# RainbowZL0/swin-unet-image-fusion

Hardware: AMD Instinct MI355X
Metric: fused image-pairs/sec at 256x256, win=8 (higher is better)
Workload: dtype bf16; 1 GPU; B=16/GPU 256x256 IR/visible pairs, win=8, 5-level Swin-UNet fusion forward (BASELINE configs[1]); global_batch=16, precision_mode=fast, residual_stream=fp32, hip_graph=True, steps_in_flight=3, kernel_schedule=throughput, collective=none, weights=random-init (numpy PCG64 recipe, seed 0)

## Files before the change

### swin_unet_image_fusion_amd/csrc/kernels_mlp.h

```cpp
#pragma once
#include "kernels_deep.h"

namespace swf {

struct MlpFusedDesc {
    const float* x[2];
    float* out[2];
    const float* gamma[2]; const float* beta[2];
    const bf16_raw* w1_hi[2]; const bf16_raw* w1_lo[2];
    const bf16_raw* w2_hi[2]; const bf16_raw* w2_lo[2];
    const float* b1[2]; const float* b2[2];
    float* scratch; int64_t scratch_floats;
    int M, C, HID;
    int schedule;
    const float* ln_gamma[2]; const float* ln_beta[2]; bf16_raw* ln_hi[2]; bf16_raw* ln_lo[2];
    const float* part0[2]; const float* part1[2]; const float* pbias[2]; float* x1[2];
};

bool mlp_fused_supported(int C, int HID);
int mlp_fused_splits(int C, int HID);
inline bool mlp_fused_writes_ln(int, int) { return true; }
int launch_mlp_fused(const MlpFusedDesc& d, int nstream, hipStream_t stream, int* route = nullptr);

}
```

### swin_unet_image_fusion_amd/csrc/kernels_mlp.hip

```cpp
#include "kernels_mlp.h"

#include <algorithm>
#include <cstdlib>

#include "win_frag.h"

#ifdef SWF_MLP_PROBE
__device__ unsigned long long swf_mlp_probe[64];
__device__ unsigned long long swf_mlp_wg[2 * 4096];
#define SWF_PROBE(i) do { if (threadIdx.x == 0) { const unsigned long long t_ = wall_clock64(); \
        if (blockIdx.x == SWF_MLP_PROBE && blockIdx.y == 0 && blockIdx.z == 0) swf_mlp_probe[i] = t_; \
        if ((i) == 0 || (i) == 41) swf_mlp_wg[2 * (((blockIdx.z * gridDim.y + blockIdx.y) * gridDim.x + blockIdx.x) & 4095) + ((i) == 41)] = t_; } } while (0)
#else
#define SWF_PROBE(i) do { } while (0)
#endif

namespace swf {

namespace {

using namespace wf;

struct MlpArgs {
    const float* x[2]; float* out[2];
    const float* gamma[2]; const float* beta[2];
    const bf16* w1_hi[2]; const bf16* w1_lo[2]; const bf16* w2_hi[2]; const bf16* w2_lo[2];
    const float* b1[2]; const float* b2[2];
    float* scratch;
    int M, HID, splits, nchunks;
    const float* ln_gamma[2]; const float* ln_beta[2]; bf16* ln_hi[2]; bf16* ln_lo[2];
    const float* part0[2]; const float* part1[2]; const float* pbias[2]; float* x1[2];
};

__device__ __forceinline__ void mma3(f32x16& acc, const bf16x8 wh, const bf16x8 wl, const bf16x8 bh, const bf16x8 bl) {
    acc = __builtin_amdgcn_mfma_f32_32x32x16_bf16(wl, bh, acc, 0, 0, 0);
    acc = __builtin_amdgcn_mfma_f32_32x32x16_bf16(wh, bl, acc, 0, 0, 0);
    acc = __builtin_amdgcn_mfma_f32_32x32x16_bf16(wh, bh, acc, 0, 0, 0);
}

template <int C, int NW, int TOK = 64>
__global__ __launch_bounds__(64 * NW) void mlp_fused_kernel(MlpArgs a) {
    constexpr int NT = 64 * NW, CW = 32 * NW;
    constexpr int NTT = TOK / 32;
    static_assert(TOK == 32 || TOK == 64, "token tile");
    constexpr int TPR = (NT / TOK == 4 || NT / TOK == 8) ? NT / TOK : 8;
    constexpr int LNT = TOK * TPR;
    static_assert(LNT <= NT, "row threads");
    constexpr int KS1 = C / 16;
    constexpr int T = C / 32;
    constexpr int NF = T / NW, R = T % NW;
    static_assert(R == 0 || 2 * R == NW, "the left-over output tiles must deal out as one half tile per wave");
    static_assert(R == 0 || NTT == 2, "half tiles need two token halves");
    constexpr int NH = R ? 1 : 0;
    constexpr int NFR = NF + NH;
    constexpr int KS2 = CW / 16;
    constexpr int NFRAG = KS1 + KS2 * NFR;
    constexpr int D = NW == 8 ? 8 : (NFRAG % 16 == 0) ? 16 : (NFRAG % 14 == 0) ? 14 : 12;
    static_assert(NFRAG % D == 0, "ring depth must divide the fragment count");
    constexpr bool ALIAS = NW == 8;
    constexpr int LDA = C + 8, LDH = CW + 8;
    static_assert(!ALIAS || LDH <= LDA, "the H image must fit the A image");
    extern __shared__ __attribute__((aligned(16))) unsigned char smem[];
    bf16* a_hi = reinterpret_cast<bf16*>(smem);
    bf16* a_lo = a_hi + TOK * LDA;
    bf16* h_hi = ALIAS ? a_hi : a_lo + TOK * LDA;
    bf16* h_lo = h_hi + TOK * LDH;

    const int tile = blockIdx.x, split = blockIdx.y, s = blockIdx.z;
    const int tid = threadIdx.x, lane = tid & 63, wave = tid >> 6;
    const int r = lane & 31, hf = lane >> 5;
    const int HID = a.HID;

    const unsigned wbytes = (unsigned)C * (unsigned)HID * 2u;
    const __amdgpu_buffer_rsrc_t r1h = __builtin_amdgcn_make_buffer_rsrc(const_cast<bf16*>(a.w1_hi[s]), 0, (int)wbytes, 0x00020000);
    const __amdgpu_buffer_rsrc_t r1l = __builtin_amdgcn_make_buffer_rsrc(const_cast<bf16*>(a.w1_lo[s]), 0, (int)wbytes, 0x00020000);
    const __amdgpu_buffer_rsrc_t r2h = __builtin_amdgcn_make_buffer_rsrc(const_cast<bf16*>(a.w2_hi[s]), 0, (int)wbytes, 0x00020000);
    const __amdgpu_buffer_rsrc_t r2l = __builtin_amdgcn_make_buffer_rsrc(const_cast<bf16*>(a.w2_lo[s]), 0, (int)wbytes, 0x00020000);
    const int loff = lane * 16;
    const int wave_u = __builtin_amdgcn_readfirstlane(wave);
    const int half_nt = T - R + (wave >> 1), half_tok = wave & 1;
    const int KSH = HID / 16;
    int w2blk[NFR];
#pragma unroll
    for (int j = 0; j < NFR; ++j) w2blk[j] = (j < NF ? wave_u + NW * j : T - R + (wave_u >> 1)) * KSH;

    bf16x8 rh[D], rl[D];
    auto frag_load = [&](int f, int hb) {
        if (f < KS1) {
            const int off = (((hb >> 5) + wave_u) * KS1 + f) * 1024;
            rh[f % D] = __builtin_bit_cast(bf16x8, __builtin_amdgcn_raw_buffer_load_b128(r1h, loff, off, 0));
            rl[f % D] = __builtin_bit_cast(bf16x8, __builtin_amdgcn_raw_buffer_load_b128(r1l, loff, off, 0));
        } else {
            const int q = f - KS1, ks = q / NFR, j = q % NFR;
            const int off = (w2blk[j] + (hb >> 4) + ks) * 1024;
            rh[f % D] = __builtin_bit_cast(bf16x8, __builtin_amdgcn_raw_buffer_load_b128(r2h, loff, off, 0));
            rl[f % D] = __builtin_bit_cast(bf16x8, __builtin_amdgcn_raw_buffer_load_b128(r2l, loff, off, 0));
        }
    };

    SWF_PROBE(0);
    const int hb0 = split * a.nchunks * CW;
    {
        const bool rowt = tid < LNT;
        const int row = rowt ? tid / TPR : 0, sub = tid % TPR;
        const int m = min(tile * TOK + row, a.M - 1);
        const float* xr = a.x[s] + (int64_t)m * C;
        constexpr int NV = C / (4 * TPR), CS = 4 * TPR;
        float4 v[NV];
        if (rowt) {
#pragma unroll
            for (int i = 0; i < NV; ++i) v[i] = *reinterpret_cast<const float4*>(xr + CS * i + 4 * sub);
            if (a.part0[s]) {
                const float* p0 = a.part0[s] + (int64_t)m * C;
                const float* p1 = a.part1[s] + (int64_t)m * C;
                float4 u0[NV], u1[NV], pb[NV];
#pragma unroll
                for (int i = 0; i < NV; ++i) {
                    u0[i] = *reinterpret_cast<const float4*>(p0 + CS * i + 4 * sub);
                    u1[i] = *reinterpret_cast<const float4*>(p1 + CS * i + 4 * sub);
                    pb[i] = *reinterpret_cast<const float4*>(a.pbias[s] + CS * i + 4 * sub);
                }
                const bool wr = split == 0 && tile * TOK + row < a.M;
#pragma unroll
                for (int i = 0; i < NV; ++i) {
                    v[i].x = ((v[i].x + pb[i].x) + u0[i].x) + u1[i].x; v[i].y = ((v[i].y + pb[i].y) + u0[i].y) + u1[i].y;
                    v[i].z = ((v[i].z + pb[i].z) + u0[i].z) + u1[i].z; v[i].w = ((v[i].w + pb[i].w) + u0[i].w) + u1[i].w;
                    if (wr) *reinterpret_cast<float4*>(a.x1[s] + (int64_t)m * C + CS * i + 4 * sub) = v[i];
                }
            }
        }
        SWF_PROBE(50);
        float* gb = reinterpret_cast<float*>(ALIAS ? a_lo + TOK * LDA : h_hi);
        float4 gbv = make_float4(0.f, 0.f, 0.f, 0.f);
        if (tid < C / 2) gbv = *reinterpret_cast<const float4*>((tid < C / 4 ? a.gamma[s] : a.beta[s] - C) + 4 * tid);
        __builtin_amdgcn_sched_barrier(0);
#pragma unroll
        for (int f = 0; f < D; ++f) frag_load(f, hb0);
        __builtin_amdgcn_sched_barrier(0);
        SWF_PROBE(51);
        if (tid < C / 2) *reinterpret_cast<float4*>(gb + 4 * tid) = gbv;
        SWF_PROBE(52);
        float mean = 0.f, rstd = 0.f;
        if (rowt) {
            float sum = 0.f;
#pragma unroll
            for (int i = 0; i < NV; ++i) sum += (v[i].x + v[i].y) + (v[i].z + v[i].w);
            sum += __shfl_xor(sum, 1);
            sum += __shfl_xor(sum, 2);
            if constexpr (TPR == 8) sum += __shfl_xor(sum, 4);
            mean = sum * (1.0f / C);
            float var = 0.f;
#pragma unroll
            for (int i = 0; i < NV; ++i) {
                const float d0 = v[i].x - mean, d1 = v[i].y - mean, d2 = v[i].z - mean, d3 = v[i].w - mean;
                var += (d0 * d0 + d1 * d1) + (d2 * d2 + d3 * d3);
            }
            var += __shfl_xor(var, 1);
            var += __shfl_xor(var, 2);
            if constexpr (TPR == 8) var += __shfl_xor(var, 4);
            rstd = 1.0f / sqrtf(var * (1.0f / C) + 1e-5f);
        }
        SWF_PROBE(53);
        __syncthreads();
        SWF_PROBE(54);
        if (rowt) {
#pragma unroll
            for (int i = 0; i < NV; ++i) {
                const int c = CS * i + 4 * sub;
                const float4 gm = *reinterpret_cast<const float4*>(gb + c), bt = *reinterpret_cast<const float4*>(gb + C + c);
                const float n[4] = {(v[i].x - mean) * rstd * gm.x + bt.x, (v[i].y - mean) * rstd * gm.y + bt.y,
                                    (v[i].z - mean) * rstd * gm.z + bt.z, (v[i].w - mean) * rstd * gm.w + bt.w};
                bf16x4 h, l;
#pragma unroll
                for (int j = 0; j < 4; ++j) { h[j] = (bf16)n[j]; l[j] = (bf16)(n[j] - (float)h[j]); }
                *reinterpret_cast<bf16x4*>(a_hi + row * LDA + c) = h;
                *reinterpret_cast<bf16x4*>(a_lo + row * LDA + c) = l;
            }
        }
    }
    __syncthreads();
    SWF_PROBE(1);

    f32x16 acc2[NTT * NF + NH];
#pragma unroll
    for (int i = 0; i < NTT * NF + NH; ++i)
#pragma unroll
        for (int e = 0; e < 16; ++e) acc2[i][e] = 0.f;

    for (int ch = 0; ch < a.nchunks; ++ch) {
        const int hb = hb0 + ch * CW;
        const int hbn = ch + 1 < a.nchunks ? hb + CW : hb;
        f32x16 acc1[NTT];
#pragma unroll
        for (int t = 0; t < NTT; ++t)
#pragma unroll
            for (int e = 0; e < 16; ++e) acc1[t][e] = 0.f;
        float4 b1v[4];
#pragma unroll
        for (int g = 0; g < 4; ++g) b1v[g] = *reinterpret_cast<const float4*>(a.b1[s] + hb + 32 * wave + 8 * g + 4 * hf);
        __builtin_amdgcn_sched_barrier(0);
        bf16x8 bh[2], bl[2];
        {
            const int ko = 8 * hf;
#pragma unroll
            for (int t = 0; t < NTT; ++t) {
                bh[t] = *reinterpret_cast<const bf16x8*>(a_hi + (32 * t + r) * LDA + ko);
                bl[t] = *reinterpret_cast<const bf16x8*>(a_lo + (32 * t + r) * LDA + ko);
            }
        }
#pragma unroll
        for (int f = 0; f < KS1; ++f) {
            const bf16x8 wh = rh[f % D], wl = rl[f % D];
            if (f + D < NFRAG) frag_load(f + D, hb);
            else frag_load(f + D - NFRAG, hbn);
            bf16x8 ch_[2], cl_[2];
#pragma unroll
            for (int t = 0; t < NTT; ++t) { ch_[t] = bh[t]; cl_[t] = bl[t]; }
            if (f + 1 < KS1) {
                const int ko = 16 * (f + 1) + 8 * hf;
#pragma unroll
                for (int t = 0; t < NTT; ++t) {
                    bh[t] = *reinterpret_cast<const bf16x8*>(a_hi + (32 * t + r) * LDA + ko);
                    bl[t] = *reinterpret_cast<const bf16x8*>(a_lo + (32 * t + r) * LDA + ko);
                }
            }
            __builtin_amdgcn_sched_barrier(0);
#pragma unroll
            for (int t = 0; t < NTT; ++t) mma3(acc1[t], wh, wl, ch_[t], cl_[t]);
            __builtin_amdgcn_sched_barrier(0);
        }
        SWF_PROBE(2 + 4 * (ch & 7));
        if constexpr (ALIAS) __syncthreads();
#pragma unroll
        for (int t = 0; t < NTT; ++t)
#pragma unroll
            for (int g = 0; g < 4; ++g) {
                const int hl = 32 * wave + 8 * g + 4 * hf;
                const float4 b = b1v[g];
                const float v[4] = {elu_fast(acc1[t][4 * g] + b.x), elu_fast(acc1[t][4 * g + 1] + b.y), elu_fast(acc1[t][4 * g + 2] + b.z),
                                    elu_fast(acc1[t][4 * g + 3] + b.w)};
                bf16x4 h, l;
#pragma unroll
                for (int j = 0; j < 4; ++j) { h[j] = (bf16)v[j]; l[j] = (bf16)(v[j] - (float)h[j]); }
                *reinterpret_cast<bf16x4*>(h_hi + (32 * t + r) * LDH + hl) = h;
                *reinterpret_cast<bf16x4*>(h_lo + (32 * t + r) * LDH + hl) = l;
            }
        SWF_PROBE(3 + 4 * (ch & 7));
        __syncthreads();
        SWF_PROBE(4 + 4 * (ch & 7));
        bf16x8 xh, xl;
        {
            const int ko = 8 * hf;
            if constexpr (NF > 0) {
#pragma unroll
                for (int t = 0; t < NTT; ++t) {
                    bh[t] = *reinterpret_cast<const bf16x8*>(h_hi + (32 * t + r) * LDH + ko);
                    bl[t] = *reinterpret_cast<const bf16x8*>(h_lo + (32 * t + r) * LDH + ko);
                }
            }
            if constexpr (NH) {
                xh = *reinterpret_cast<const bf16x8*>(h_hi + (32 * half_tok + r) * LDH + ko);
                xl = *reinterpret_cast<const bf16x8*>(h_lo + (32 * half_tok + r) * LDH + ko);
            }
        }
#pragma unroll
        for (int ks = 0; ks < KS2; ++ks) {
            bf16x8 wh[NFR], wl[NFR];
#pragma unroll
            for (int j = 0; j < NFR; ++j) {
                const int f = KS1 + ks * NFR + j;
                wh[j] = rh[f % D]; wl[j] = rl[f % D];
                if (f + D < NFRAG) frag_load(f + D, hb);
                else frag_load(f + D - NFRAG, hbn);
            }
            bf16x8 ch_[2], cl_[2];
#pragma unroll
            for (int t = 0; t < NTT; ++t) { ch_[t] = bh[t]; cl_[t] = bl[t]; }
            const bf16x8 cxh = xh, cxl = xl;
            if (ks + 1 < KS2) {
                const int ko = 16 * (ks + 1) + 8 * hf;
                if constexpr (NF > 0) {
#pragma unroll
                    for (int t = 0; t < NTT; ++t) {
                        bh[t] = *reinterpret_cast<const bf16x8*>(h_hi + (32 * t + r) * LDH + ko);
                        bl[t] = *reinterpret_cast<const bf16x8*>(h_lo + (32 * t + r) * LDH + ko);
                    }
                }
                if constexpr (NH) {
                    xh = *reinterpret_cast<const bf16x8*>(h_hi + (32 * half_tok + r) * LDH + ko);
                    xl = *reinterpret_cast<const bf16x8*>(h_lo + (32 * half_tok + r) * LDH + ko);
                }
            }
            __builtin_amdgcn_sched_barrier(0);
#pragma unroll
            for (int j = 0; j < NFR; ++j) {
                if (j < NF) {
#pragma unroll
                    for (int t = 0; t < NTT; ++t) mma3(acc2[NTT * j + t], wh[j], wl[j], ch_[t], cl_[t]);
                } else {
                    mma3(acc2[NTT * NF], wh[j], wl[j], cxh, cxl);
                }
            }
            __builtin_amdgcn_sched_barrier(0);
        }
        SWF_PROBE(5 + 4 * (ch & 7));
        __syncthreads();
    }

    SWF_PROBE(40);
    constexpr int ORS = C + 4;
    static_assert(TOK * ORS * 4 <= 2 * TOK * LDA * 2, "out tile must fit the A image");
    float* otile = reinterpret_cast<float*>(smem);
    float* part = a.splits > 1 ? a.scratch + ((int64_t)(s * a.splits + split) * a.M) * C : nullptr;
    const int erow = tid < LNT ? tid / TPR : 0, esub = tid % TPR;
    const int em = tile * TOK + erow;
    const bool live = !part && em < a.M && tid < LNT;
    constexpr int ENV = C / (4 * TPR), ECS = 4 * TPR;
    float4 exr[ENV], eb2[ENV], eg[ENV], ebt[ENV];
    const bool ln_out = !part && a.ln_hi[s] != nullptr;
    if (live) {
        const float* xres = (a.part0[s] ? a.x1[s] : a.x[s]) + (int64_t)em * C;
#pragma unroll
        for (int i = 0; i < ENV; ++i) {
            const int c = ECS * i + 4 * esub;
            exr[i] = *reinterpret_cast<const float4*>(xres + c);
            eb2[i] = *reinterpret_cast<const float4*>(a.b2[s] + c);
        }
        if (ln_out) {
#pragma unroll
            for (int i = 0; i < ENV; ++i) {
                const int c = ECS * i + 4 * esub;
                eg[i] = *reinterpret_cast<const float4*>(a.ln_gamma[s] + c);
                ebt[i] = *reinterpret_cast<const float4*>(a.ln_beta[s] + c);
            }
        }
    }
    __builtin_amdgcn_sched_barrier(0);
#pragma unroll
    for (int i = 0; i < NTT * NF + NH; ++i) {
        const int nt = i < NTT * NF ? wave + NW * (i / NTT) : half_nt;
        const int t = i < NTT * NF ? (i % NTT) : half_tok;
#pragma unroll
        for (int g = 0; g < 4; ++g)
            *reinterpret_cast<float4*>(otile + (32 * t + r) * ORS + 32 * nt + 8 * g + 4 * hf) =
                make_float4(acc2[i][4 * g], acc2[i][4 * g + 1], acc2[i][4 * g + 2], acc2[i][4 * g + 3]);
    }
    __syncthreads();
    constexpr int C4 = C / 4;
    if (part) {
#pragma unroll 4
        for (int idx = tid; idx < TOK * C4; idx += NT) {
            const int row = idx / C4, c = (idx % C4) * 4;
            const int m = tile * TOK + row;
            if (m >= a.M) continue;
            *reinterpret_cast<float4*>(part + (int64_t)m * C + c) = *reinterpret_cast<const float4*>(otile + row * ORS + c);
        }
    } else {
        float4 v[ENV];
        float sum = 0.f;
#pragma unroll
        for (int i = 0; i < ENV; ++i) {
            const int c = ECS * i + 4 * esub;
            v[i] = make_float4(0.f, 0.f, 0.f, 0.f);
            if (live) {
                float4 t = *reinterpret_cast<const float4*>(otile + erow * ORS + c);
                const float4 b = eb2[i], x = exr[i];
                t.x += b.x + x.x; t.y += b.y + x.y; t.z += b.z + x.z; t.w += b.w + x.w;
                *reinterpret_cast<float4*>(a.out[s] + (int64_t)em * C + c) = t;
                v[i] = t;
            }
            sum += (v[i].x + v[i].y) + (v[i].z + v[i].w);
        }
        if (ln_out) {
            sum += __shfl_xor(sum, 1);
            sum += __shfl_xor(sum, 2);
            if constexpr (TPR == 8) sum += __shfl_xor(sum, 4);
            const float mean = sum * (1.0f / C);
            float q = 0.f;
#pragma unroll
            for (int i = 0; i < ENV; ++i) {
                const float d0 = v[i].x - mean, d1 = v[i].y - mean, d2 = v[i].z - mean, d3 = v[i].w - mean;
                q += (d0 * d0 + d1 * d1) + (d2 * d2 + d3 * d3);
            }
            q += __shfl_xor(q, 1);
            q += __shfl_xor(q, 2);
            if constexpr (TPR == 8) q += __shfl_xor(q, 4);
            const float rstd = 1.0f / sqrtf(q * (1.0f / C) + 1e-5f);
            if (live) {
#pragma unroll
                for (int i = 0; i < ENV; ++i) {
                    const int c = ECS * i + 4 * esub;
                    const float4 g = eg[i], b = ebt[i];
                    const float n[4] = {(v[i].x - mean) * rstd * g.x + b.x, (v[i].y - mean) * rstd * g.y + b.y,
                                        (v[i].z - mean) * rstd * g.z + b.z, (v[i].w - mean) * rstd * g.w + b.w};
                    bf16x4 hi, lo;
#pragma unroll
                    for (int j = 0; j < 4; ++j) { hi[j] = (bf16)n[j]; lo[j] = (bf16)(n[j] - (float)hi[j]); }
                    *reinterpret_cast<bf16x4*>(a.ln_hi[s] + (int64_t)em * C + c) = hi;
                    *reinterpret_cast<bf16x4*>(a.ln_lo[s] + (int64_t)em * C + c) = lo;
                }
            }
        }
    }
    SWF_PROBE(41);
}

__global__ __launch_bounds__(256) void mlp_reduce_kernel(MlpArgs a, int C) {
    const int s = blockIdx.y;
    const int64_t total = (int64_t)a.M * C, total4 = total >> 2;
    const float* part = a.scratch + (int64_t)s * a.splits * total;
    for (int64_t e4 = (int64_t)blockIdx.x * blockDim.x + threadIdx.x; e4 < total4; e4 += (int64_t)gridDim.x * blockDim.x) {
        const int64_t e = e4 << 2;
        const int c = (int)(e % C);
        float4 v = *reinterpret_cast<const float4*>(part + e);
        for (int k = 1; k < a.splits; ++k) {
            const float4 t = *reinterpret_cast<const float4*>(part + k * total + e);
            v.x += t.x; v.y += t.y; v.z += t.z; v.w += t.w;
        }
        const float4 b = *reinterpret_cast<const float4*>(a.b2[s] + c);
        const float4 x = *reinterpret_cast<const float4*>(a.x[s] + e);
        v.x += b.x + x.x; v.y += b.y + x.y; v.z += b.z + x.z; v.w += b.w + x.w;
        *reinterpret_cast<float4*>(a.out[s] + e) = v;
    }
}

template <int NCH>
__global__ __launch_bounds__(256) void mlp_reduce_ln_kernel(MlpArgs a, int C, int L) {
    const int s = blockIdx.y;
    const int64_t gt = (int64_t)blockIdx.x * blockDim.x + threadIdx.x;
    const int64_t tok = gt / L;
    const int sub = (int)(gt % L);
    const bool live = tok < a.M;
    const int chunks = C >> 2;
    const int64_t total = (int64_t)a.M * C, row = (live ? tok : 0) * C;
    const float* part = a.scratch + (int64_t)s * a.splits * total + row;
    float4 v[NCH], gm[NCH], bt[NCH];
    float sum = 0.f;
#pragma unroll
    for (int i = 0; i < NCH; ++i) {
        const int ch = sub + i * L;
        v[i] = gm[i] = bt[i] = make_float4(0.f, 0.f, 0.f, 0.f);
        if (live && ch < chunks) {
            float4 u[6];
#pragma unroll
            for (int k = 0; k < 6; ++k)
                u[k] = k < a.splits ? *reinterpret_cast<const float4*>(part + k * total + 4 * ch) : make_float4(0.f, 0.f, 0.f, 0.f);
            const float4 b = *reinterpret_cast<const float4*>(a.b2[s] + 4 * ch);
            const float4 x = *reinterpret_cast<const float4*>(a.x[s] + row + 4 * ch);
            gm[i] = *reinterpret_cast<const float4*>(a.ln_gamma[s] + 4 * ch);
            bt[i] = *reinterpret_cast<const float4*>(a.ln_beta[s] + 4 * ch);
            float4 t = u[0];
#pragma unroll
            for (int k = 1; k < 6; ++k)
                if (k < a.splits) { t.x += u[k].x; t.y += u[k].y; t.z += u[k].z; t.w += u[k].w; }
            for (int k = 6; k < a.splits; ++k) {
                const float4 w = *reinterpret_cast<const float4*>(part + k * total + 4 * ch);
                t.x += w.x; t.y += w.y; t.z += w.z; t.w += w.w;
            }
            t.x += b.x + x.x; t.y += b.y + x.y; t.z += b.z + x.z; t.w += b.w + x.w;
            *reinterpret_cast<float4*>(a.out[s] + row + 4 * ch) = t;
            v[i] = t;
        }
        sum += (v[i].x + v[i].y) + (v[i].z + v[i].w);
    }
    for (int o = L >> 1; o > 0; o >>= 1) sum += __shfl_xor(sum, o);
    const float mean = sum / (float)C;
    float q = 0.f;
#pragma unroll
    for (int i = 0; i < NCH; ++i) {
        if (sub + i * L < chunks) {
            const float d0 = v[i].x - mean, d1 = v[i].y - mean, d2 = v[i].z - mean, d3 = v[i].w - mean;
            q += (d0 * d0 + d1 * d1) + (d2 * d2 + d3 * d3);
        }
    }
    for (int o = L >> 1; o > 0; o >>= 1) q += __shfl_xor(q, o);
    const float rstd = 1.0f / sqrtf(q / (float)C + 1e-5f);
    if (!live) return;
#pragma unroll
    for (int i = 0; i < NCH; ++i) {
        const int ch = sub + i * L;
        if (ch < chunks) {
            const float4 g = gm[i], b = bt[i];
            const float r[4] = {(v[i].x - mean) * rstd * g.x + b.x, (v[i].y - mean) * rstd * g.y + b.y,
                                (v[i].z - mean) * rstd * g.z + b.z, (v[i].w - mean) * rstd * g.w + b.w};
            bf16x4 hi, lo;
#pragma unroll
            for (int j = 0; j < 4; ++j) { hi[j] = (bf16)r[j]; lo[j] = (bf16)(r[j] - (float)hi[j]); }
            *reinterpret_cast<bf16x4*>(a.ln_hi[s] + row + 4 * ch) = hi;
            *reinterpret_cast<bf16x4*>(a.ln_lo[s] + row + 4 * ch) = lo;
        }
    }
}

template <int C, int NW, int TOK = 64>
int launch_c(const MlpArgs& a, int nstream, hipStream_t stream, int* route) {
    constexpr int lds = NW == 8 ? TOK * (C + 8) * 2 * 2 + 2 * C * 4 : (TOK * (C + 8) + TOK * (32 * NW + 8)) * 2 * 2;
    if (NW == 8 && a.nchunks != 1) return fail(SWF_ERR_UNSUPPORTED, "mlp_fused: the 8-wave kernel takes one hidden chunk per workgroup");
    if (lds > 65536) SWF_TRY((raise_lds_limit<&mlp_fused_kernel<C, NW, TOK>>(lds, "mlp_fused")));
    dim3 grid((a.M + TOK - 1) / TOK, a.splits, nstream);
    hipLaunchKernelGGL((mlp_fused_kernel<C, NW, TOK>), grid, dim3(64 * NW), lds, stream, a);
    SWF_TRY(check_launch("mlp_fused"));
    trace_block(route, NW == 8 ? SWF_BLOCK_MLP_WIDE8 : TOK == 32 ? SWF_BLOCK_MLP_TOK32 : SWF_BLOCK_MLP_TOK64);
    if (a.splits > 1) trace_block(route, SWF_BLOCK_MLP_SPLIT);
    MlpArgs ra = a;
    for (int s = 0; s < nstream; ++s)
        if (a.part0[s]) ra.x[s] = a.x1[s];
    if (a.splits > 1 && a.ln_hi[0]) {
        constexpr int chunks = C / 4, L = chunks > 32 ? 64 : 32, NCH = (chunks + L - 1) / L;
        dim3 rgrid((unsigned)cdiv64((int64_t)a.M * L, 256), nstream);
        hipLaunchKernelGGL((mlp_reduce_ln_kernel<NCH>), rgrid, dim3(256), 0, stream, ra, C, L);
        return check_launch("mlp_reduce_ln");
    }
    if (a.splits > 1) {
        dim3 rgrid((unsigned)std::min<int64_t>(cdiv64((int64_t)a.M * C, 1024), 2048), nstream);
        hipLaunchKernelGGL(mlp_reduce_kernel, rgrid, dim3(256), 0, stream, ra, C);
        return check_launch("mlp_reduce");
    }
    return SWF_OK;
}

}

static bool mlp_wide(int C, int HID) {
    static const bool off = [] { const char* e = debug_env("SWF_MLP8"); return e && e[0] == '0'; }();
    return !off && C == 384 && HID % 256 == 0;
}

static bool mlp_tok32(int C, int HID) {
    static const bool off = [] { const char* e = debug_env("SWF_MLP_TOK32"); return e && e[0] == '0'; }();
    return !off && C == 192 && HID % 192 == 0;
}

bool mlp_fused_supported(int C, int HID) {
    return (C == 128 || C == 192 || C == 256 || C == 384) && HID > 0 && HID % 128 == 0 && (int64_t)C * HID < (1 << 30);
}

int mlp_fused_splits(int C, int HID) {
    static const int forced = [] { const char* e = debug_env("SWF_MLP_SPLITS"); return e ? atoi(e) : 0; }();
    if (mlp_wide(C, HID)) return HID / 256;
    if (mlp_tok32(C, HID)) return 1;
    if (forced > 0 && (HID / 128) % forced == 0) return forced;
    const int chunks = HID / 128;
    if (C <= 256) return chunks % 2 == 0 ? 2 : 1;
    return chunks % 2 == 0 ? chunks / 2 : chunks;
}

int launch_mlp_fused(const MlpFusedDesc& d, int nstream, hipStream_t stream, int* route) {
    if (!mlp_fused_supported(d.C, d.HID)) return fail(SWF_ERR_UNSUPPORTED, "mlp_fused: C=%d hidden=%d", d.C, d.HID);
    if (d.M <= 0 || d.M > (1 << 30) / d.C) return fail(SWF_ERR_UNSUPPORTED, "mlp_fused: token count %d", d.M);
    MlpArgs a{};
    for (int s = 0; s < nstream; ++s) {
        a.x[s] = d.x[s]; a.out[s] = d.out[s]; a.gamma[s] = d.gamma[s]; a.beta[s] = d.beta[s];
        a.w1_hi[s] = reinterpret_cast<const bf16*>(d.w1_hi[s]); a.w1_lo[s] = reinterpret_cast<const bf16*>(d.w1_lo[s]);
        a.w2_hi[s] = reinterpret_cast<const bf16*>(d.w2_hi[s]); a.w2_lo[s] = reinterpret_cast<const bf16*>(d.w2_lo[s]);
        a.b1[s] = d.b1[s]; a.b2[s] = d.b2[s];
    }
    if (d.part0[0]) {
        for (int s = 0; s < nstream; ++s) {
            if (!d.part0[s] || !d.part1[s] || !d.pbias[s] || !d.x1[s]) return fail(SWF_ERR_NULL, "mlp_fused: attention-tail inputs must be given for every stream");
            if (d.x1[s] == d.x[s] || d.x1[s] == d.out[s]) return fail(SWF_ERR_UNSUPPORTED, "mlp_fused: x1 must not alias x / out");
            a.part0[s] = d.part0[s]; a.part1[s] = d.part1[s]; a.pbias[s] = d.pbias[s]; a.x1[s] = d.x1[s];
        }
    }
    a.M = d.M; a.HID = d.HID;
    a.splits = mlp_fused_splits(d.C, d.HID);
    const bool wide = mlp_wide(d.C, d.HID), tok32 = mlp_tok32(d.C, d.HID) && d.schedule != SWF_SCHED_THROUGHPUT;
    a.nchunks = d.HID / (wide ? 256 : tok32 ? 192 : 128) / a.splits;
    a.scratch = d.scratch;
    if (d.ln_hi[0])
        for (int s = 0; s < nstream; ++s) {
            a.ln_gamma[s] = d.ln_gamma[s]; a.ln_beta[s] = d.ln_beta[s];
            a.ln_hi[s] = reinterpret_cast<bf16*>(d.ln_hi[s]); a.ln_lo[s] = reinterpret_cast<bf16*>(d.ln_lo[s]);
        }
    if (a.splits > 1 && (!d.scratch || (int64_t)nstream * a.splits * d.M * d.C > d.scratch_floats))
        return fail(SWF_ERR_WORKSPACE, "mlp_fused: scratch too small for %d hidden splits", a.splits);
    switch (d.C) {
        case 128: return launch_c<128, 4>(a, nstream, stream, route);
        case 192: return tok32 ? launch_c<192, 6, 32>(a, nstream, stream, route) : launch_c<192, 4>(a, nstream, stream, route);
        case 256: return launch_c<256, 4>(a, nstream, stream, route);
        case 384: return wide ? launch_c<384, 8>(a, nstream, stream, route) : launch_c<384, 4>(a, nstream, stream, route);
    }
    return fail(SWF_ERR_UNSUPPORTED, "mlp_fused: C=%d", d.C);
}

}
```

### swin_unet_image_fusion_amd/csrc/kernels_qkvattn.h

```cpp
#pragma once
#include "kernels_deep.h"

namespace swf {

bool qkvattn_supported(const swf_block_desc& d);
size_t qkvattn_packed_bytes(const swf_block_desc& d);
int pack_qkvattn(const swf_block_desc& d, const swf_block_stream_params& p, void* dst, hipStream_t stream);

struct QkvAttnArgs {
    const void* packed[2];
    const bf16_raw* xn_hi[2]; const bf16_raw* xn_lo[2];
    bf16_raw* o_hi[2]; bf16_raw* o_lo[2];
    float* part[2][2];
    int B, H, W, shift, cross;
};
int launch_qkvattn(const swf_block_desc& d, const QkvAttnArgs& a, int nstream, hipStream_t stream);

}
```

### swin_unet_image_fusion_amd/csrc/kernels_qkvattn.hip

```cpp
#include "kernels_qkvattn.h"

#include <algorithm>

#include "win_frag.h"

namespace swf {
namespace {

using namespace wf;

template <int C_>
struct QA {
    static constexpr int C = C_, D = 24, HEADS = 8, HG = 4, KS = C / 16;
    static constexpr int NFRAG = HEADS * 3 * KS * 2;
    static constexpr size_t p_bvec = size_t(NFRAG) * 1024;
    static constexpr size_t p_bias = p_bvec + size_t(HEADS) * 3 * 32 * 4;
    static constexpr size_t p_proj = p_bias + size_t(2) * 2 * 16 * 64 * 4;
    static constexpr int NT = C / 32, NPF = (HEADS / HG) * NT * HG * 2 * 2;
    static constexpr size_t p_total = p_proj + size_t(NPF) * 1024;
    static constexpr int XS = C * 2 + 16;
    static constexpr size_t l_plane = size_t(64) * XS, l_tile = 2 * l_plane;
    static constexpr size_t l_xq = 0, l_xkv = l_tile, l_k = 2 * l_tile, l_v = l_k + HG * 4 * 1024, l_total = l_v + HG * 4 * 1024;
    static_assert(XS % 16 == 0 && (XS / 16) % 2 == 1, "row stride must be an odd number of 16-byte slots");
    static_assert(l_total <= 160 * 1024, "LDS");
};

struct QaDev {
    const char* packed[2];
    const bf16* xn_hi[2]; const bf16* xn_lo[2];
    bf16* o_hi[2]; bf16* o_lo[2];
    float* part[2][2];
    int B, H, W, shift, cross, nstream;
};

#ifdef QA_PROBE
__device__ unsigned long long qa_probe[8];
#define QA_STAMP(i) do { if (blockIdx.x == QA_PROBE && blockIdx.y == 0 && blockIdx.z == 0 && threadIdx.x == 0) qa_probe[i] = wall_clock64(); } while (0)
#else
#define QA_STAMP(i) do { } while (0)
#endif

template <int C, int WS>
__global__ __launch_bounds__(512, 2) void qkv_attn_kernel(QaDev a) {
    using G = QA<C>;
    static_assert(WS == 7 || WS == 8, "window side");
    constexpr int KS = G::KS, XS = G::XS;
    extern __shared__ __attribute__((aligned(16))) char smem[];
    u32x4* kimg = reinterpret_cast<u32x4*>(smem + G::l_k);
    u32x4* vimg = reinterpret_cast<u32x4*>(smem + G::l_v);

    const int tid = threadIdx.x, lane = tid & 63, wave = tid >> 6;
    const int hl = wave >> 1, tt = wave & 1, r = lane & 31, hf = lane >> 5;
    const int H = a.H, W = a.W, nwx = W / WS, nwy = H / WS, npi = nwx * nwy;
    const int win = blockIdx.x, st = blockIdx.y, hg = blockIdx.z, head = hg * G::HG + hl;
    const int b = win / npi, wrem = win - b * npi, wy = wrem / nwx, wx = wrem - wy * nwx;
    const int sh = a.shift ? WS / 2 : 0;
    const bool cross = a.cross && a.nstream == 2;
    const int kvs = cross ? 1 - st : st;

    auto tok_index = [&](int t) {
        int oy = wy * WS + (t >> 3) + sh, ox = wx * WS + (t & 7) + sh;
        oy = oy >= H ? oy - H : oy;
        ox = ox >= W ? ox - W : ox;
        return (b * H + oy) * W + ox;
    };

    QA_STAMP(0);
    const __amdgpu_buffer_rsrc_t wrs = __builtin_amdgcn_make_buffer_rsrc(const_cast<char*>(uniform_ptr(a.packed[st])), 0, (int)G::p_total, 0x00020000);
    const unsigned loff = (unsigned)lane * 16u;
    const int fbase = head * 3 * KS * 2;
    auto WFRAG = [&](int m, int s, int hl2) {
        return __builtin_bit_cast(u32x4, __builtin_amdgcn_raw_buffer_load_b128(wrs, loff, ((fbase + (m * KS + s) * 2 + hl2)) * 1024, 0));
    };
    constexpr int PD = 4;
    u32x4 w[PD][6];
#pragma unroll
    for (int p = 0; p < PD && p < KS; ++p)
#pragma unroll
        for (int m = 0; m < 3; ++m) { w[p][2 * m] = WFRAG(m, p, 0); w[p][2 * m + 1] = WFRAG(m, p, 1); }

    {
        constexpr int CPR = C / 8, NCH = 2 * 64 * CPR, PER = NCH / 512;
        static_assert(NCH % 512 == 0, "chunks per tile must divide evenly over the workgroup");
        const int ntile = cross ? 2 : 1;
        for (int tile = 0; tile < ntile; ++tile) {
            const int s_src = tile ? kvs : st;
            u32x4 v[PER];
            int dst[PER];
#pragma unroll
            for (int i = 0; i < PER; ++i) {
                const int rem = tid + 512 * i, plane = rem / (64 * CPR), rem2 = rem - plane * 64 * CPR;
                const int row = rem2 / CPR, j = rem2 - row * CPR;
                const bf16* src = (plane ? a.xn_lo[s_src] : a.xn_hi[s_src]) + (int64_t)tok_index(row) * C + j * 8;
                v[i] = *reinterpret_cast<const u32x4*>(src);
                dst[i] = tile * (int)G::l_tile + plane * (int)G::l_plane + row * XS + j * 16;
            }
#pragma unroll
            for (int i = 0; i < PER; ++i) *reinterpret_cast<u32x4*>(smem + dst[i]) = v[i];
        }
    }
    __syncthreads();
    QA_STAMP(1);

    const char* xq = smem + G::l_xq + (32 * tt + r) * XS + hf * 16;
    const char* xk = smem + (cross ? G::l_xkv : G::l_xq) + (32 * tt + r) * XS + hf * 16;
    const f32x16 zero16 = {0.f, 0.f, 0.f, 0.f, 0.f, 0.f, 0.f, 0.f, 0.f, 0.f, 0.f, 0.f, 0.f, 0.f, 0.f, 0.f};
    f32x16 aq = zero16, ak = zero16, av = zero16;
    {
#pragma unroll
        for (int s = 0; s < KS; ++s) {
            SWF_WF_FENCE();
            const u32x4 xh = *reinterpret_cast<const u32x4*>(xq + s * 32), xl = *reinterpret_cast<const u32x4*>(xq + G::l_plane + s * 32);
            u32x4 kh = xh, kl = xl;
            if (cross) {
                kh = *reinterpret_cast<const u32x4*>(xk + s * 32);
                kl = *reinterpret_cast<const u32x4*>(xk + G::l_plane + s * 32);
            }
            u32x4 (&ws_)[6] = w[s % PD];
            aq = mma3(ws_[0], ws_[1], xh, xl, aq);
            ak = mma3(ws_[2], ws_[3], kh, kl, ak);
            av = mma3(kh, kl, ws_[4], ws_[5], av);
            SWF_WF_FENCE();
            if (s + PD < KS) {
#pragma unroll
                for (int m = 0; m < 3; ++m) { ws_[2 * m] = WFRAG(m, s + PD, 0); ws_[2 * m + 1] = WFRAG(m, s + PD, 1); }
            }
        }
    }
    QA_STAMP(2);
    u32x4 qf[2];
    {
        const float* bvec = reinterpret_cast<const float*>(a.packed[st] + G::p_bvec) + head * 3 * 32;
        float t[16];
#pragma unroll
        for (int g = 0; g < 4; ++g) {
            const float4 bq = *reinterpret_cast<const float4*>(bvec + 8 * g + 4 * hf);
            t[4 * g] = aq[4 * g] + bq.x; t[4 * g + 1] = aq[4 * g + 1] + bq.y; t[4 * g + 2] = aq[4 * g + 2] + bq.z; t[4 * g + 3] = aq[4 * g + 3] + bq.w;
        }
        qf[0] = pack8_f16(t);
        qf[1] = pack8_f16(t + 8);
#pragma unroll
        for (int g = 0; g < 4; ++g) {
            const float4 bk = *reinterpret_cast<const float4*>(bvec + 32 + 8 * g + 4 * hf);
            t[4 * g] = ak[4 * g] + bk.x; t[4 * g + 1] = ak[4 * g + 1] + bk.y; t[4 * g + 2] = ak[4 * g + 2] + bk.z; t[4 * g + 3] = ak[4 * g + 3] + bk.w;
        }
        u32x4* kdst = kimg + ((hl * 2 + tt) * 2) * 64 + lane;
        kdst[0] = pack8_f16(t);
        kdst[64] = pack8_f16(t + 8);
        const float bv = bvec[64 + r];
#pragma unroll
        for (int i = 0; i < 16; ++i) t[i] = av[i] + bv;
        u32x4* vdst = vimg + (hl * 4 + 2 * tt) * 64 + lane;
        vdst[0] = pack8_f16(t);
        vdst[64] = pack8_f16(t + 8);
    }
    __syncthreads();
    QA_STAMP(3);

    const int qt = tt;
    f32x16 bias[2];
    {
        const float* bm = reinterpret_cast<const float*>(a.packed[st] + G::p_bias) + qt * 2 * 16 * 64 + lane;
#pragma unroll
        for (int kt = 0; kt < 2; ++kt)
#pragma unroll
            for (int i = 0; i < 16; ++i) bias[kt][i] = bm[(kt * 16 + i) * 64];
    }
    const bool rowv = a.shift && wy == nwy - 1, colv = a.shift && wx == nwx - 1;
    const bool col_masked = (hf != 0) != (((r >> 2) & 1) != 0);
    const bool m0 = (rowv && qt == 1) || (colv && col_masked), m1 = (rowv && qt == 0) || (colv && col_masked);
    const u32x4* ksrc = kimg + (hl * 4) * 64 + lane;
    const u32x4* vsrc = vimg + (hl * 4) * 64 + lane;
    const u32x4 k00 = ksrc[0], k01 = ksrc[64], k10 = ksrc[128], k11 = ksrc[192];
    f32x16 s0 = mfma_f16(k00, qf[0], bias[0]);
    s0 = mfma_f16(k01, qf[1], s0);
    f32x16 s1 = mfma_f16(k10, qf[0], bias[1]);
    s1 = mfma_f16(k11, qf[1], s1);
    if (rowv || colv) {
#pragma unroll
        for (int i = 0; i < 16; ++i) {
            s0[i] = m0 ? -INFINITY : s0[i];
            s1[i] = m1 ? -INFINITY : s1[i];
        }
    }
    float mx = max3f(s0[0], s0[1], s1[0]);
    mx = max3f(mx, s1[1], s0[2]);
#pragma unroll
    for (int i = 3; i < 16; i += 2) mx = max3f(mx, s0[i], s0[i + 1 < 16 ? i + 1 : i]);
#pragma unroll
    for (int i = 2; i < 16; i += 2) mx = max3f(mx, s1[i], s1[i + 1]);
    {
        float lo, hi;
        halves(mx, lo, hi);
        mx = __builtin_fmaxf(lo, hi);
    }
    {
        const f16 nm = (f16)(-mx);
        u32x4 q1 = qf[1];
        q1[2] |= hf == 0 ? (unsigned)__builtin_bit_cast(unsigned short, nm) : 0u;
        s0 = mfma_f16(k00, qf[0], bias[0]);
        s0 = mfma_f16(k01, q1, s0);
        s1 = mfma_f16(k10, qf[0], bias[1]);
        s1 = mfma_f16(k11, q1, s1);
    }
    if (rowv || colv) {
#pragma unroll
        for (int i = 0; i < 16; ++i) {
            s0[i] = m0 ? -INFINITY : s0[i];
            s1[i] = m1 ? -INFINITY : s1[i];
        }
    }
    f32x16 t;
#pragma unroll
    for (int ps = 0; ps < 4; ++ps) {
        float p[8];
#pragma unroll
        for (int j = 0; j < 8; ++j) p[j] = __builtin_amdgcn_exp2f((ps >> 1) ? s1[8 * (ps & 1) + j] : s0[8 * (ps & 1) + j]);
        t = mfma_f16(vsrc[ps * 64], pack8_f16(p), ps == 0 ? zero16 : t);
    }
    QA_STAMP(4);
    float den, unused;
    halves(t[12], den, unused);
    const float inv = __builtin_amdgcn_rcpf(den);
    auto padding = [](int t) { return WS != 8 && ((t >> 3) >= WS || (t & 7) >= WS); };
    if (a.part[0][st] == nullptr) {
        if (padding(32 * qt + r)) return;
        const int64_t orow = (int64_t)tok_index(32 * qt + r) * (G::HEADS * G::D) + head * G::D + 4 * hf;
        bf16* oh = a.o_hi[st] + orow;
        bf16* ol = a.o_lo[st] + orow;
#pragma unroll
        for (int g = 0; g < 3; ++g) {
            bf16x4 h4, l4;
#pragma unroll
            for (int j = 0; j < 4; ++j) {
                const float v = t[4 * g + j] * inv;
                h4[j] = (bf16)v;
                l4[j] = (bf16)(v - (float)h4[j]);
            }
            *reinterpret_cast<bf16x4*>(oh + 8 * g) = h4;
            *reinterpret_cast<bf16x4*>(ol + 8 * g) = l4;
        }
    } else {
        constexpr int NT = G::NT;
        const int pbase = (int)(G::p_proj / 1024) + hg * NT * G::HG * 4;
        auto PFRAG = [&](int tile, int f) {
            return __builtin_bit_cast(u32x4, __builtin_amdgcn_raw_buffer_load_b128(wrs, loff, (pbase + tile * G::HG * 4 + f) * 1024, 0));
        };
        u32x4 wp[G::HG * 4];
#pragma unroll
        for (int f = 0; f < G::HG * 4; ++f) wp[f] = PFRAG(hl, f);
        float ov[16];
#pragma unroll
        for (int i = 0; i < 16; ++i) ov[i] = t[i] * inv;
        u32x4* ofr = reinterpret_cast<u32x4*>(smem + G::l_xq);
        {
            u32x4 h0, l0, h1, l1;
            split8(ov, h0, l0);
            split8(ov + 8, h1, l1);
            u32x4* dst = ofr + ((hl * 2 + tt) * 4) * 64 + lane;
            dst[0] = h0; dst[64] = l0; dst[128] = h1; dst[192] = l1;
        }
        __syncthreads();
        int tokrow[16];
#pragma unroll
        for (int i = 0; i < 16; ++i) tokrow[i] = tok_index(32 * tt + rho(i, hf)) * C;
        float* pout = a.part[hg][st];
        for (int tile = hl; tile < NT; tile += G::HG) {
            f32x16 acc = zero16;
#pragma unroll
            for (int h2 = 0; h2 < G::HG; ++h2)
#pragma unroll
                for (int ks = 0; ks < 2; ++ks) {
                    const u32x4* src = ofr + ((h2 * 2 + tt) * 4 + 2 * ks) * 64 + lane;
                    acc = mma3(src[0], src[64], wp[(h2 * 2 + ks) * 2], wp[(h2 * 2 + ks) * 2 + 1], acc);
                }
            if (tile + G::HG < NT) {
#pragma unroll
                for (int f = 0; f < G::HG * 4; ++f) wp[f] = PFRAG(tile + G::HG, f);
            }
#pragma unroll
            for (int i = 0; i < 16; ++i)
                if (!padding(32 * tt + rho(i, hf))) pout[tokrow[i] + 32 * tile + r] = acc[i];
        }
    }
    QA_STAMP(5);
}

struct QaPackArgs { swf_attn_params p; char* dst; int ws; };

template <int C>
__global__ __launch_bounds__(256) void qa_pack_kernel(QaPackArgs a) {
    using G = QA<C>;
    const int gtid = blockIdx.x * blockDim.x + threadIdx.x, gsz = gridDim.x * blockDim.x;
    const float qscale = kLog2e / sqrtf((float)G::D);
    for (int idx = gtid; idx < G::NFRAG * 512; idx += gsz) {
        const int f = idx >> 9, lane = (idx >> 3) & 63, e = idx & 7, r = lane & 31, hf = lane >> 5;
        const int hl = f & 1, s = (f >> 1) % G::KS, m = (f / (2 * G::KS)) % 3, head = f / (6 * G::KS);
        const swf_linear& l = m == 0 ? a.p.q : m == 1 ? a.p.k : a.p.v;
        float val = 0.f;
        if (r < G::D) {
            val = l.weight[(int64_t)(head * G::D + r) * C + s * 16 + 8 * hf + e];
            if (m == 0) val *= qscale;
        }
        const bf16 hi = (bf16)val;
        reinterpret_cast<bf16*>(a.dst)[idx] = hl ? (bf16)(val - (float)hi) : hi;
    }
    bf16* pf = reinterpret_cast<bf16*>(a.dst + G::p_proj);
    for (int idx = gtid; idx < G::NPF * 512; idx += gsz) {
        const int f = idx >> 9, lane = (idx >> 3) & 63, e = idx & 7, r = lane & 31, hf = lane >> 5;
        const int hl = f & 1, ks = (f >> 1) & 1, h2 = (f >> 2) % G::HG, tile = (f / (4 * G::HG)) % G::NT, hg = f / (4 * G::HG * G::NT);
        const int vc = rho(8 * ks + e, hf);
        float val = 0.f;
        if (vc < G::D) val = a.p.proj.weight[(int64_t)(32 * tile + r) * (G::HEADS * G::D) + (hg * G::HG + h2) * G::D + vc];
        const bf16 hi = (bf16)val;
        pf[idx] = hl ? (bf16)(val - (float)hi) : hi;
    }
    float* bvec = reinterpret_cast<float*>(a.dst + G::p_bvec);
    for (int i = gtid; i < G::HEADS * 3 * 32; i += gsz) {
        const int c = i & 31, m = (i >> 5) % 3, head = i / 96;
        const swf_linear& l = m == 0 ? a.p.q : m == 1 ? a.p.k : a.p.v;
        float v = 0.f;
        if (c < G::D) v = (l.bias ? l.bias[head * G::D + c] : 0.f) * (m == 0 ? qscale : 1.0f);
        else if (c == G::D && m != 0) v = 1.0f;
        bvec[i] = v;
    }
    float* bm = reinterpret_cast<float*>(a.dst + G::p_bias);
    for (int i = gtid; i < 2 * 2 * 16 * 64; i += gsz) {
        const int lane = i & 63, reg = (i >> 6) & 15, kt = (i >> 10) & 1, qt = i >> 11;
        const int key = 32 * kt + rho(reg, lane >> 5), q = 32 * qt + (lane & 31);
        const int ky = key >> 3, kx = key & 7, qy = q >> 3, qx = q & 7, ws = a.ws, tw = 2 * ws - 1;
        float v = 0.f;
        if (ky >= ws || kx >= ws) v = -INFINITY;
        else if (qy < ws && qx < ws) v = a.p.bias_table[(ky - qy + ws - 1) * tw + (kx - qx + ws - 1)] * kLog2e;
        bm[i] = v;
    }
}

}

bool qkvattn_supported(const swf_block_desc& d) {
    return d.precision == SWF_PREC_FAST && d.attn.channels == 192 && d.attn.heads == 8 && d.attn.head_dim == 24 && d.attn.win_h == d.attn.win_w &&
           (d.attn.win_h == 8 || d.attn.win_h == 7);
}

size_t qkvattn_packed_bytes(const swf_block_desc& d) { return qkvattn_supported(d) ? align_up(QA<192>::p_total, 256) : 0; }

int pack_qkvattn(const swf_block_desc& d, const swf_block_stream_params& p, void* dst, hipStream_t stream) {
    if (!qkvattn_supported(d)) return fail(SWF_ERR_UNSUPPORTED, "pack_qkvattn: shape not covered");
    QaPackArgs a{p.attn, static_cast<char*>(dst), d.attn.win_h};
    hipLaunchKernelGGL((qa_pack_kernel<192>), dim3(128), dim3(256), 0, stream, a);
    return check_launch("pack_qkvattn");
}

int launch_qkvattn(const swf_block_desc& d, const QkvAttnArgs& a, int nstream, hipStream_t stream) {
    const int wsd = d.attn.win_h;
    if (!qkvattn_supported(d) || a.H % wsd || a.W % wsd) return fail(SWF_ERR_UNSUPPORTED, "qkvattn: shape not covered");
    using G = QA<192>;
    QaDev dv{};
    for (int s = 0; s < nstream; ++s) {
        dv.packed[s] = static_cast<const char*>(a.packed[s]);
        dv.xn_hi[s] = reinterpret_cast<const bf16*>(a.xn_hi[s]); dv.xn_lo[s] = reinterpret_cast<const bf16*>(a.xn_lo[s]);
        dv.o_hi[s] = reinterpret_cast<bf16*>(a.o_hi[s]); dv.o_lo[s] = reinterpret_cast<bf16*>(a.o_lo[s]);
        dv.part[0][s] = a.part[0][s]; dv.part[1][s] = a.part[1][s];
    }
    if ((dv.part[0][0] != nullptr) != (dv.part[1][0] != nullptr) || (nstream == 2 && (dv.part[0][1] != nullptr) != (dv.part[0][0] != nullptr)))
        return fail(SWF_ERR_NULL, "qkvattn: projection partial buffers must be given for both head groups and streams or not at all");
    dv.B = a.B; dv.H = a.H; dv.W = a.W; dv.shift = a.shift; dv.cross = a.cross; dv.nstream = nstream;
    const int nwin = a.B * (a.H / wsd) * (a.W / wsd);
    if (wsd == 8) {
        SWF_TRY((raise_lds_limit<&qkv_attn_kernel<192, 8>>((int)G::l_total, "qkv_attn")));
        hipLaunchKernelGGL((qkv_attn_kernel<192, 8>), dim3(nwin, nstream, 2), dim3(512), G::l_total, stream, dv);
    } else {
        SWF_TRY((raise_lds_limit<&qkv_attn_kernel<192, 7>>((int)G::l_total, "qkv_attn")));
        hipLaunchKernelGGL((qkv_attn_kernel<192, 7>), dim3(nwin, nstream, 2), dim3(512), G::l_total, stream, dv);
    }
    return check_launch("qkv_attn");
}

}
```

### swin_unet_image_fusion_amd/csrc/swf_api.hip

```cpp
#include <algorithm>
#include <cmath>
#include <mutex>
#include <string>
#include <vector>

#include "kernels_generic.h"
#include <cstdlib>
#include "kernels_window.h"
#include "kernels_bwd.h"
#include "kernels_dropout.h"
#include "kernels_loss.h"
#include "kernels_fidelity.h"
#include "kernels_structure.h"
#include "kernels_metrics.h"
#include "kernels_optim.h"
#include "kernels_deep.h"
#include "kernels_patch.h"
#include "kernels_patchrr.h"
#include "kernels_deeppatch.h"
#include "kernels_mlp.h"
#include "kernels_qkvattn.h"
#include "kernels_attnproj.h"

namespace swf {

char* err_buf() {
    static thread_local char buf[512] = "";
    return buf;
}
int fail(int status, const char* fmt, ...) {
    va_list ap;
    va_start(ap, fmt);
    vsnprintf(err_buf(), 512, fmt, ap);
    va_end(ap);
    return status;
}

static int check_attn_desc(const swf_attn_desc* d, int B, int H, int W) {
    if (!d) return fail(SWF_ERR_NULL, "desc is NULL");
    if (d->channels <= 0 || d->heads <= 0 || d->head_dim <= 0 || d->win_h <= 0 || d->win_w <= 0)
        return fail(SWF_ERR_BAD_SHAPE, "non-positive attention dims");
    if (B <= 0 || H <= 0 || W <= 0) return fail(SWF_ERR_BAD_SHAPE, "empty batch or map (%d,%d,%d)", B, H, W);
    if (H % d->win_h || W % d->win_w)
        return fail(SWF_ERR_BAD_SHAPE, "map %dx%d is not a multiple of the window %dx%d", H, W, d->win_h, d->win_w);
    return SWF_OK;
}

static int64_t splitk_need(int K, int64_t nprob_m_n) {
    const int sk = gemm_splitk_for(K);
    return sk > 1 ? sk * nprob_m_n : 0;
}

struct AttnBufs { float *qkv[2][3], *o[2], *sk, *bias16; int64_t sk_floats; };
static AttnBufs carve_attention(Carver& ws, const swf_attn_desc& d, int nstream, int64_t N, int fast) {
    const int C = d.channels, HD = d.heads * d.head_dim;
    AttnBufs b{};
    for (int s = 0; s < nstream; ++s) {
        for (int i = 0; i < 3; ++i) b.qkv[s][i] = ws.floats(N * HD);
        b.o[s] = ws.floats(N * HD);
    }
    b.sk_floats = fast ? std::max(splitk_need(C, 3 * nstream * N * HD), splitk_need(HD, nstream * N * C)) : 0;
    b.sk = fast ? ws.floats(b.sk_floats) : nullptr;
    const bool win16 = fast && attn_core_mfma16_supported(d.win_h, d.win_w, d.head_dim);
    b.bias16 = win16 ? ws.floats((int64_t)attn_core_mfma16_scratch_floats(nstream)) : nullptr;
    return b;
}

static int attention_generic(const swf_attn_desc& d, int nstream, const swf_attn_params* const* prm,
                             const float* const* qsrc, const float* const* ksrc, const float* const* vsrc,
                             const float* const* residual, float* const* out, int B, int H, int W, const AttnBufs& bufs,
                             hipStream_t stream, int fast = 0, const swf_norm* const* qnorm = nullptr,
                             const swf_norm* const* kvnorm = nullptr) {
    const int64_t N = (int64_t)B * H * W;
    const int C = d.channels, HD = d.heads * d.head_dim;
    GemmBatch gb{};
    gb.scratch = bufs.sk; gb.scratch_floats = bufs.sk_floats;
    for (int s = 0; s < nstream; ++s) {
        const swf_linear* lin[3] = {&prm[s]->q, &prm[s]->k, &prm[s]->v};
        const float* src[3] = {qsrc[s], ksrc[s], vsrc[s]};
        for (int i = 0; i < 3; ++i) gb.p[s * 3 + i] = GemmProb{src[i], lin[i]->weight, lin[i]->bias, nullptr, bufs.qkv[s][i]};
    }
    if (qnorm) {
        LnGemmBatch lb{};
        for (int s = 0; s < nstream; ++s) {
            const swf_linear* lin[3] = {&prm[s]->q, &prm[s]->k, &prm[s]->v};
            const float* src[3] = {qsrc[s], ksrc[s], vsrc[s]};
            const swf_norm* nrm[3] = {qnorm[s], kvnorm[s], kvnorm[s]};
            for (int i = 0; i < 3; ++i) lb.p[s * 3 + i] = LnGemmProb{src[i], nrm[i]->gamma, nrm[i]->beta, lin[i]->weight, lin[i]->bias, bufs.qkv[s][i]};
        }
        SWF_TRY(launch_lngemm_bf16x3(lb, nstream * 3, (int)N, HD, C, 0, stream));
    } else {
        SWF_TRY(launch_gemm(fast, gb, nstream * 3, (int)N, HD, C, C, HD, 0, stream));
    }
    if (bufs.bias16) {
        const float* qq[2] = {bufs.qkv[0][0], bufs.qkv[1][0]};
        const float* kk[2] = {bufs.qkv[0][1], bufs.qkv[1][1]};
        const float* vv[2] = {bufs.qkv[0][2], bufs.qkv[1][2]};
        const float* tt[2] = {prm[0]->bias_table, nstream == 2 ? prm[1]->bias_table : nullptr};
        SWF_TRY(launch_attn_core_mfma16(qq, kk, vv, bufs.o, tt, nstream, HD, HD, HD, HD, B, H, W, d.heads, d.head_dim, d.shift, bufs.bias16, stream));
    } else if (fast && attn_core_mfma_supported(d.win_h, d.win_w, d.head_dim)) {
        const float* qq[2] = {bufs.qkv[0][0], bufs.qkv[1][0]};
        const float* kk[2] = {bufs.qkv[0][1], bufs.qkv[1][1]};
        const float* vv[2] = {bufs.qkv[0][2], bufs.qkv[1][2]};
        const float* tt[2] = {prm[0]->bias_table, nstream == 2 ? prm[1]->bias_table : nullptr};
        SWF_TRY(launch_attn_core_mfma(qq, kk, vv, bufs.o, tt, nstream, HD, HD, HD, HD, B, H, W, d.heads, d.head_dim, d.shift, stream, nullptr, nullptr,
                                      nullptr, nullptr, nullptr, d.win_h));
    } else {
        AttnCoreBatch ab{};
        for (int s = 0; s < nstream; ++s) ab.p[s] = AttnCoreProb{bufs.qkv[s][0], bufs.qkv[s][1], bufs.qkv[s][2], bufs.o[s], prm[s]->bias_table};
        SWF_TRY(launch_attn_core(ab, nstream, HD, HD, HD, HD, B, H, W, d.win_h, d.win_w, d.heads, d.head_dim, d.shift, stream));
    }
    GemmBatch pb{};
    pb.scratch = bufs.sk; pb.scratch_floats = bufs.sk_floats;
    for (int s = 0; s < nstream; ++s)
        pb.p[s] = GemmProb{bufs.o[s], prm[s]->proj.weight, prm[s]->proj.bias, residual ? residual[s] : nullptr, out[s]};
    SWF_TRY(launch_gemm(fast, pb, nstream, (int)N, C, HD, HD, C, 0, stream));
    return SWF_OK;
}

static size_t attention_generic_ws(const swf_attn_desc& d, int nstream, int B, int H, int W) {
    Carver exact = Carver::measure(), fast = Carver::measure();
    carve_attention(exact, d, nstream, (int64_t)B * H * W, 0);
    carve_attention(fast, d, nstream, (int64_t)B * H * W, 1);
    return std::max(exact.bytes(), fast.bytes());
}

static int check_stream_params(const swf_block_stream_params* p, const char* which, bool need_attn, bool need_mlp) {
    if (!p) return fail(SWF_ERR_NULL, "%s params are NULL", which);
    if (need_attn && (!p->ln1.gamma || !p->ln1.beta || !p->attn.q.weight || !p->attn.k.weight || !p->attn.v.weight ||
                      !p->attn.proj.weight || !p->attn.bias_table))
        return fail(SWF_ERR_NULL, "%s: attention half has a NULL weight", which);
    if (need_mlp && (!p->ln2.gamma || !p->ln2.beta || !p->fc1.weight || !p->fc2.weight))
        return fail(SWF_ERR_NULL, "%s: MLP half has a NULL weight", which);
    return SWF_OK;
}

struct AttnHalfBufs { float* xn[2]; AttnBufs a; };
static AttnHalfBufs carve_attn_half(Carver& ws, const swf_block_desc& d, int nstream, int64_t N) {
    const int fast = d.precision == SWF_PREC_FAST;
    AttnHalfBufs b{};
    if (!(fast && lngemm_supported(d.attn.channels)))
        for (int s = 0; s < nstream; ++s) b.xn[s] = ws.floats(N * d.attn.channels);
    b.a = carve_attention(ws, d.attn, nstream, N, fast);
    return b;
}

static int attn_halfblock_generic(const swf_block_desc* desc, const swf_block_stream_params* px,
                                  const swf_block_stream_params* py, const float* x_in, const float* y_in, float* x_out,
                                  float* y_out, int B, int H, int W, Carver& ws, hipStream_t stream) {
    const int nstream = py ? 2 : 1;
    const int64_t N = (int64_t)B * H * W;
    const int C = desc->attn.channels;
    const bool cross = desc->cross && nstream == 2;
    const int fast = desc->precision == SWF_PREC_FAST;
    const swf_attn_params* prm[2] = {&px->attn, py ? &py->attn : nullptr};
    const float* res[2] = {x_in, y_in};
    float* out[2] = {x_out, y_out};
    const AttnHalfBufs bufs = carve_attn_half(ws, *desc, nstream, N);
    if (!ws.ok()) return fail(SWF_ERR_WORKSPACE, "attention half-block workspace too small (need %zu B)", ws.bytes());
    if (fast && lngemm_supported(C)) {
        const float* raw[2] = {x_in, y_in};
        const swf_norm* nrm[2] = {&px->ln1, py ? &py->ln1 : nullptr};
        const float* qsrc[2] = {raw[0], raw[1]};
        const float* kvsrc[2] = {cross ? raw[1] : raw[0], cross ? raw[0] : raw[1]};
        const swf_norm* kvn[2] = {cross ? nrm[1] : nrm[0], cross ? nrm[0] : nrm[1]};
        return attention_generic(desc->attn, nstream, prm, qsrc, kvsrc, kvsrc, res, out, B, H, W, bufs.a, stream, fast, nrm, kvn);
    }
    float* const* xn = bufs.xn;
    LnBatch lb{};
    lb.p[0] = LnProb{x_in, xn[0], px->ln1.gamma, px->ln1.beta};
    if (nstream == 2) lb.p[1] = LnProb{y_in, xn[1], py->ln1.gamma, py->ln1.beta};
    SWF_TRY(launch_layernorm(lb, nstream, N, C, 0, stream));
    const float* qsrc[2] = {xn[0], xn[1]};
    const float* kvsrc[2] = {cross ? xn[1] : xn[0], cross ? xn[0] : xn[1]};
    return attention_generic(desc->attn, nstream, prm, qsrc, kvsrc, kvsrc, res, out, B, H, W, bufs.a, stream, fast);
}

struct MlpHalfBufs { float *xn[2], *hb[2], *sk; int64_t sk_floats; };
static MlpHalfBufs carve_mlp_half(Carver& ws, const swf_block_desc& d, int nstream, int64_t N) {
    const int C = d.attn.channels, hid = d.hidden;
    const int fast = d.precision == SWF_PREC_FAST;
    MlpHalfBufs b{};
    if (!(fast && lngemm_supported(C)))
        for (int s = 0; s < nstream; ++s) b.xn[s] = ws.floats(N * C);
    for (int s = 0; s < nstream; ++s) b.hb[s] = ws.floats(N * hid);
    b.sk_floats = fast ? std::max(splitk_need(C, nstream * N * hid), splitk_need(hid, nstream * N * C)) : 0;
    b.sk = fast ? ws.floats(b.sk_floats) : nullptr;
    return b;
}

static int mlp_halfblock_generic(const swf_block_desc* desc, const swf_block_stream_params* px,
                                 const swf_block_stream_params* py, const float* x_in, const float* y_in, float* x_out,
                                 float* y_out, int B, int H, int W, Carver& ws, hipStream_t stream) {
    const int nstream = py ? 2 : 1;
    const int64_t N = (int64_t)B * H * W;
    const int C = desc->attn.channels, hid = desc->hidden;
    const int fast = desc->precision == SWF_PREC_FAST;
    const bool fold_ln = fast && lngemm_supported(C);
    const MlpHalfBufs bufs = carve_mlp_half(ws, *desc, nstream, N);
    if (!ws.ok()) return fail(SWF_ERR_WORKSPACE, "MLP half-block workspace too small (need %zu B)", ws.bytes());
    const swf_block_stream_params* pp[2] = {px, py};
    const float* res[2] = {x_in, y_in};
    float* out[2] = {x_out, y_out};
    GemmBatch g2{};
    g2.scratch = bufs.sk; g2.scratch_floats = bufs.sk_floats;
    for (int s = 0; s < nstream; ++s) g2.p[s] = GemmProb{bufs.hb[s], pp[s]->fc2.weight, pp[s]->fc2.bias, res[s], out[s]};
    if (fold_ln) {
        LnGemmBatch l1{};
        for (int s = 0; s < nstream; ++s) l1.p[s] = LnGemmProb{res[s], pp[s]->ln2.gamma, pp[s]->ln2.beta, pp[s]->fc1.weight, pp[s]->fc1.bias, bufs.hb[s]};
        SWF_TRY(launch_lngemm_bf16x3(l1, nstream, (int)N, hid, C, 1, stream));
    } else {
        LnBatch lb{};
        lb.p[0] = LnProb{x_in, bufs.xn[0], px->ln2.gamma, px->ln2.beta};
        if (nstream == 2) lb.p[1] = LnProb{y_in, bufs.xn[1], py->ln2.gamma, py->ln2.beta};
        SWF_TRY(launch_layernorm(lb, nstream, N, C, 0, stream));
        GemmBatch g1{};
        g1.scratch = bufs.sk; g1.scratch_floats = bufs.sk_floats;
        for (int s = 0; s < nstream; ++s) g1.p[s] = GemmProb{bufs.xn[s], pp[s]->fc1.weight, pp[s]->fc1.bias, nullptr, bufs.hb[s]};
        SWF_TRY(launch_gemm(fast, g1, nstream, (int)N, hid, C, C, hid, 1, stream));
    }
    SWF_TRY(launch_gemm(fast, g2, nstream, (int)N, C, hid, hid, C, 0, stream));
    return SWF_OK;
}

static void deep_ln1_planes(Carver& ws, int64_t N, int C, int nstream, bf16_raw** hi, bf16_raw** lo) {
    for (int s = 0; s < nstream; ++s) {
        hi[s] = reinterpret_cast<bf16_raw*>(ws.floats(N * C / 2));
        lo[s] = reinterpret_cast<bf16_raw*>(ws.floats(N * C / 2));
    }
}

struct DeepBufs {
    bf16_raw *xn_hi[2], *xn_lo[2], *o_hi[2], *o_lo[2], *h_hi[2], *h_lo[2];
    bf16_raw* qkv[2][3];
    void* wbuf[2];
    float *sk, *part[2][2], *x1[2];
    int64_t sk_floats;
};
static DeepBufs carve_deep_block(Carver& ws, const swf_block_desc& d, int nstream, int64_t N, bool fused_mlp) {
    const int C = d.attn.channels, HD = d.attn.heads * d.attn.head_dim, hid = d.hidden;
    auto planes = [&](int64_t n) { return reinterpret_cast<bf16_raw*>(ws.floats(n / 2)); };
    DeepBufs b{};
    deep_ln1_planes(ws, N, C, nstream, b.xn_hi, b.xn_lo);
    for (int s = 0; s < nstream; ++s) {
        b.wbuf[s] = ws.floats((int64_t)deep_block_packed_bytes(d) / 4);
        for (int i = 0; i < 3; ++i) b.qkv[s][i] = planes(N * HD);
        b.o_hi[s] = planes(N * HD); b.o_lo[s] = planes(N * HD);
        b.h_hi[s] = planes(N * hid); b.h_lo[s] = planes(N * hid);
    }
    int64_t skn = std::max((int64_t)gemm_sp_splitk_for(HD, SP_EPI_F32), (int64_t)gemm_sp_splitk_for(hid, SP_EPI_F32));
    if (fused_mlp) skn = std::max(skn, (int64_t)mlp_fused_splits(C, hid));
    b.sk_floats = skn > 1 ? skn * nstream * N * C : 0;
    b.sk = ws.floats(b.sk_floats);
    if (qkvattn_supported(d) && mlp_fused_supported(C, hid) && HD == C)
        for (int s = 0; s < nstream; ++s) { b.part[0][s] = ws.floats(N * C); b.part[1][s] = ws.floats(N * C); b.x1[s] = ws.floats(N * C); }
    return b;
}
static size_t deep_block_ws(const swf_block_desc* d, int nstream, int B, int H, int W) {
    if (!deep_block_supported(*d)) return 0;
    Carver plain = Carver::measure(), fused = Carver::measure();
    carve_deep_block(plain, *d, nstream, (int64_t)B * H * W, false);
    carve_deep_block(fused, *d, nstream, (int64_t)B * H * W, mlp_fused_supported(d->attn.channels, d->hidden));
    return std::max(plain.bytes(), fused.bytes());
}

static size_t block_generic_ws(const swf_block_desc* d, int nstream, int B, int H, int W) {
    Carver a = Carver::measure(), m = Carver::measure();
    carve_attn_half(a, *d, nstream, (int64_t)B * H * W);
    carve_mlp_half(m, *d, nstream, (int64_t)B * H * W);
    return std::max(std::max(a.bytes(), m.bytes()), deep_block_ws(d, nstream, B, H, W));
}

static int deep_block_impl(const swf_block_desc* desc, const swf_block_stream_params* px, const swf_block_stream_params* py,
                           const float* x_in, const float* y_in, float* x_out, float* y_out, int B, int H, int W,
                           Carver& ws, hipStream_t stream, const void* packed_x, const void* packed_y,
                           const swf_block_stream_params* const* next_p = nullptr, bool* ln1_ready = nullptr, int* route = nullptr) {
    const bool ln1_given = ln1_ready && *ln1_ready;
    if (ln1_ready) *ln1_ready = false;
    const int nstream = py ? 2 : 1;
    const int64_t N = (int64_t)B * H * W;
    const int C = desc->attn.channels, HD = desc->attn.heads * desc->attn.head_dim, hid = desc->hidden;
    const bool cross = desc->cross && nstream == 2;
    const swf_block_stream_params* pp[2] = {px, py};
    const float* xin[2] = {x_in, y_in};
    float* xout[2] = {x_out, y_out};
    const void* pk[2] = {packed_x, packed_y};
    static const bool no_fused_mlp = debug_env("SWF_NO_FUSED_MLP") != nullptr;
    const bool fused_mlp = !no_fused_mlp && mlp_fused_supported(C, hid) && N <= INT32_MAX / 2;
    const DeepBufs b = carve_deep_block(ws, *desc, nstream, N, fused_mlp);
    if (!ws.ok()) return fail(SWF_ERR_WORKSPACE, "deep block workspace too small (need %zu B)", ws.bytes());
    static const bool no_qkvattn = debug_env("SWF_NO_QKVATTN") != nullptr;
    static const bool no_projfuse = debug_env("SWF_NO_PROJFUSE") != nullptr;
    const bool fused_attn_shape = !no_qkvattn && qkvattn_supported(*desc) && N <= INT32_MAX / 256;
    const bool proj_fused = fused_attn_shape && fused_mlp && !no_projfuse && HD == C && (int64_t)H * W <= 256;
    DeepWeights wv[2];
    trace_block(route, SWF_BLOCK_ROUTE_DEEP);
    if (pk[0] && (nstream == 1 || pk[1])) trace_block(route, SWF_BLOCK_PREPACKED);
    for (int s = 0; s < nstream; ++s) {
        if (!pk[s]) { SWF_TRY(pack_deep_block(*desc, *pp[s], b.wbuf[s], stream)); pk[s] = b.wbuf[s]; }
        wv[s] = deep_block_views(*desc, pk[s]);
    }
    if (!ln1_given) {
        LnBatch l1{};
        for (int s = 0; s < nstream; ++s) l1.p[s] = LnProb{xin[s], nullptr, pp[s]->ln1.gamma, pp[s]->ln1.beta, b.xn_hi[s], b.xn_lo[s]};
        SWF_TRY(launch_layernorm(l1, nstream, N, C, 0, stream));
    } else {
        trace_block(route, SWF_BLOCK_LN1_GIVEN);
    }
    const bool fused_attn = fused_attn_shape && wv[0].qa && (nstream == 1 || wv[1].qa);
    const bool fold_proj = proj_fused && fused_attn && pp[0]->attn.proj.bias && (nstream == 1 || pp[1]->attn.proj.bias);
    if (fused_attn) {
        QkvAttnArgs qa{};
        for (int s = 0; s < nstream; ++s) {
            qa.packed[s] = wv[s].qa; qa.xn_hi[s] = b.xn_hi[s]; qa.xn_lo[s] = b.xn_lo[s]; qa.o_hi[s] = b.o_hi[s]; qa.o_lo[s] = b.o_lo[s];
            if (fold_proj) { qa.part[0][s] = b.part[0][s]; qa.part[1][s] = b.part[1][s]; }
        }
        qa.B = B; qa.H = H; qa.W = W; qa.shift = desc->attn.shift; qa.cross = cross;
        SWF_TRY(launch_qkvattn(*desc, qa, nstream, stream));
        trace_block(route, SWF_BLOCK_DEEP_QKVATTN | (fold_proj ? SWF_BLOCK_DEEP_FOLD_PROJ : 0));
    }
    SpGemmBatch gq{};
    for (int s = 0; s < nstream; ++s) {
        const int kvs = cross ? 1 - s : s;
        const swf_linear* lin[3] = {&pp[s]->attn.q, &pp[s]->attn.k, &pp[s]->attn.v};
        const bf16_raw* wh[3] = {wv[s].q_hi, wv[s].k_hi, wv[s].v_hi};
        const bf16_raw* wl[3] = {wv[s].q_lo, wv[s].k_lo, wv[s].v_lo};
        for (int i = 0; i < 3; ++i) {
            const int src = i == 0 ? s : kvs;
            gq.p[s * 3 + i] = SpGemmProb{b.xn_hi[src], b.xn_lo[src], wh[i], wl[i], lin[i]->bias, nullptr, nullptr, b.qkv[s][i], nullptr};
        }
    }
    gq.qscale = 1.4426950408889634f / std::sqrt((float)desc->attn.head_dim);
    const bool deep_qkv = !fused_attn && HD == C && deep_qkv_supported(*desc) && wv[0].qkvf_hi && (nstream == 1 || wv[1].qkvf_hi);
    if (deep_qkv) {
        DeepQkvArgs dq{};
        for (int s = 0; s < nstream; ++s) {
            dq.xn_hi[s] = b.xn_hi[s]; dq.xn_lo[s] = b.xn_lo[s]; dq.w_hi[s] = wv[s].qkvf_hi; dq.w_lo[s] = wv[s].qkvf_lo;
            dq.bias[s][0] = pp[s]->attn.q.bias; dq.bias[s][1] = pp[s]->attn.k.bias; dq.bias[s][2] = pp[s]->attn.v.bias;
            for (int i = 0; i < 3; ++i) dq.out[s][i] = b.qkv[s][i];
        }
        dq.qscale = gq.qscale; dq.cross = cross; dq.M = (int)N; dq.C = C; dq.schedule = desc->schedule;
        SWF_TRY(launch_deep_qkv(dq, nstream, stream));
        trace_block(route, SWF_BLOCK_DEEP_QKV);
    }
    if (!fused_attn && !deep_qkv) SWF_TRY(launch_gemm_sp(gq, 3 * nstream, (int)N, HD, C, HD, SP_EPI_QKV16, stream));
    const bool attn_proj = !fused_attn && HD == C && attnproj_supported(*desc) && wv[0].pf_hi && (nstream == 1 || wv[1].pf_hi);
    if (attn_proj) {
        AttnProjArgs ap{};
        for (int s = 0; s < nstream; ++s) {
            ap.q[s] = b.qkv[s][0]; ap.k[s] = b.qkv[s][1]; ap.v[s] = b.qkv[s][2];
            ap.wp_hi[s] = wv[s].pf_hi; ap.wp_lo[s] = wv[s].pf_lo; ap.pbias[s] = pp[s]->attn.proj.bias; ap.table[s] = pp[s]->attn.bias_table;
            ap.res[s] = xin[s]; ap.out[s] = xout[s];
        }
        ap.B = B; ap.H = H; ap.W = W; ap.shift = desc->attn.shift;
        SWF_TRY(launch_attnproj(*desc, ap, nstream, stream));
        trace_block(route, SWF_BLOCK_DEEP_ATTNPROJ);
    }
    if (!fused_attn && !attn_proj) {
        const bf16_raw* qq[2] = {b.qkv[0][0], b.qkv[1][0]};
        const bf16_raw* kk[2] = {b.qkv[0][1], b.qkv[1][1]};
        const bf16_raw* vv[2] = {b.qkv[0][2], b.qkv[1][2]};
        const float* tt[2] = {pp[0]->attn.bias_table, nstream == 2 ? pp[1]->attn.bias_table : nullptr};
        if (desc->attn.win_h == 16) {
            SWF_TRY(launch_attn_core_mfma16(nullptr, nullptr, nullptr, nullptr, tt, nstream, HD, HD, HD, HD, B, H, W, desc->attn.heads,
                                            desc->attn.head_dim, desc->attn.shift, nullptr, stream, b.o_hi, b.o_lo, qq, kk, vv));
            trace_block(route, SWF_BLOCK_DEEP_CORE16);
        } else
            SWF_TRY(launch_attn_core_mfma(nullptr, nullptr, nullptr, nullptr, tt, nstream, HD, HD, HD, HD, B, H, W, desc->attn.heads,
                                          desc->attn.head_dim, desc->attn.shift, stream, b.o_hi, b.o_lo, qq, kk, vv, desc->attn.win_h));
    }
    SpGemmBatch gp{};
    gp.scratch = b.sk; gp.scratch_floats = b.sk_floats;
    for (int s = 0; s < nstream; ++s)
        gp.p[s] = SpGemmProb{b.o_hi[s], b.o_lo[s], wv[s].p_hi, wv[s].p_lo, pp[s]->attn.proj.bias, xin[s], xout[s], nullptr, nullptr};
    const bool deep_proj = !fold_proj && !attn_proj && HD == C && deep_proj_supported(*desc) && wv[0].pf_hi && (nstream == 1 || wv[1].pf_hi);
    if (deep_proj) {
        DeepProjArgs dp{};
        for (int s = 0; s < nstream; ++s) {
            dp.o_hi[s] = b.o_hi[s]; dp.o_lo[s] = b.o_lo[s]; dp.w_hi[s] = wv[s].pf_hi; dp.w_lo[s] = wv[s].pf_lo;
            dp.bias[s] = pp[s]->attn.proj.bias; dp.res[s] = xin[s]; dp.out[s] = xout[s];
        }
        dp.M = (int)N; dp.C = C;
        SWF_TRY(launch_deep_proj(dp, nstream, stream));
        trace_block(route, SWF_BLOCK_DEEP_PROJ);
    }
    if (!fold_proj && !attn_proj && !deep_proj) SWF_TRY(launch_gemm_sp(gp, nstream, (int)N, C, HD, C, SP_EPI_F32, stream));
    if (fused_mlp) {
        MlpFusedDesc md{};
        for (int s = 0; s < nstream; ++s) {
            md.x[s] = fold_proj ? xin[s] : xout[s]; md.out[s] = xout[s]; md.gamma[s] = pp[s]->ln2.gamma; md.beta[s] = pp[s]->ln2.beta;
            if (fold_proj) { md.part0[s] = b.part[0][s]; md.part1[s] = b.part[1][s]; md.pbias[s] = pp[s]->attn.proj.bias; md.x1[s] = b.x1[s]; }
            md.w1_hi[s] = wv[s].w1f_hi; md.w1_lo[s] = wv[s].w1f_lo; md.w2_hi[s] = wv[s].w2f_hi; md.w2_lo[s] = wv[s].w2f_lo;
            md.b1[s] = pp[s]->fc1.bias; md.b2[s] = pp[s]->fc2.bias;
        }
        md.scratch = b.sk; md.scratch_floats = b.sk_floats; md.M = (int)N; md.C = C; md.HID = hid; md.schedule = desc->schedule;
        const bool ln_next = next_p && ln1_ready && next_p[0] && (nstream == 1 || next_p[1]) && mlp_fused_writes_ln(C, hid);
        if (ln_next)
            for (int s = 0; s < nstream; ++s) {
                md.ln_gamma[s] = next_p[s]->ln1.gamma; md.ln_beta[s] = next_p[s]->ln1.beta; md.ln_hi[s] = b.xn_hi[s]; md.ln_lo[s] = b.xn_lo[s];
            }
        trace_block(route, SWF_BLOCK_MLP_FUSED);
        SWF_TRY(launch_mlp_fused(md, nstream, stream, route));
        if (ln_next) { *ln1_ready = true; trace_block(route, SWF_BLOCK_LN1_WRITTEN); }
        return SWF_OK;
    }
    LnBatch l2{};
    for (int s = 0; s < nstream; ++s) l2.p[s] = LnProb{xout[s], nullptr, pp[s]->ln2.gamma, pp[s]->ln2.beta, b.xn_hi[s], b.xn_lo[s]};
    SWF_TRY(launch_layernorm(l2, nstream, N, C, 0, stream));
    SpGemmBatch g1{};
    for (int s = 0; s < nstream; ++s)
        g1.p[s] = SpGemmProb{b.xn_hi[s], b.xn_lo[s], wv[s].w1_hi, wv[s].w1_lo, pp[s]->fc1.bias, nullptr, nullptr, b.h_hi[s], b.h_lo[s]};
    SWF_TRY(launch_gemm_sp(g1, nstream, (int)N, hid, C, hid, SP_EPI_ELU_SPLIT, stream));
    SpGemmBatch g2{};
    g2.scratch = b.sk; g2.scratch_floats = b.sk_floats;
    for (int s = 0; s < nstream; ++s)
        g2.p[s] = SpGemmProb{b.h_hi[s], b.h_lo[s], wv[s].w2_hi, wv[s].w2_lo, pp[s]->fc2.bias, xout[s], xout[s], nullptr, nullptr};
    return launch_gemm_sp(g2, nstream, (int)N, C, hid, C, SP_EPI_F32, stream);
}

static size_t block_packed_bytes(const swf_block_desc& d) {
    const size_t pb = window_block_packed_bytes(d);
    return pb ? pb : deep_block_packed_bytes(d);
}

static int check_block(const swf_block_desc* desc, const swf_block_stream_params* px, const swf_block_stream_params* py,
                       const float* x_in, const float* y_in, float* x_out, float* y_out, int B, int H, int W,
                       bool attn, bool mlp) {
    if (!desc) return fail(SWF_ERR_NULL, "desc is NULL");
    SWF_TRY(check_attn_desc(&desc->attn, B, H, W));
    if (mlp && desc->hidden <= 0) return fail(SWF_ERR_BAD_SHAPE, "hidden must be positive");
    SWF_TRY(check_stream_params(px, "x-stream", attn, mlp));
    if (!x_in || !x_out) return fail(SWF_ERR_NULL, "x tensors are NULL");
    if (py) {
        SWF_TRY(check_stream_params(py, "y-stream", attn, mlp));
        if (!y_in || !y_out) return fail(SWF_ERR_NULL, "y tensors are NULL with dual-path params");
    }
    return SWF_OK;
}

struct WindowBufs { char* packed; float *ox, *oy; };
static WindowBufs carve_window_block(Carver& ws, const swf_block_desc& d, int64_t N, bool prepacked, bool tmp_out) {
    WindowBufs b{};
    if (!prepacked) b.packed = reinterpret_cast<char*>(ws.floats((int64_t)(2 * window_block_packed_bytes(d) / 4)));
    if (tmp_out) {
        b.ox = ws.floats(2 * N * d.attn.channels);
        b.oy = b.ox ? b.ox + N * d.attn.channels : nullptr;
    }
    return b;
}
static size_t window_block_ws(const swf_block_desc& d, int B, int H, int W) {
    if (!window_block_supported(d, B, H, W)) return 0;
    size_t need = 0;
    for (int route = 0; route < 4; ++route) {
        if ((route & 2) && !window_block_out_of_place(d)) continue;
        Carver m = Carver::measure();
        carve_window_block(m, d, (int64_t)B * H * W, (route & 1) != 0, (route & 2) != 0);
        need = std::max(need, m.bytes());
    }
    return need;
}

static int basic_block_impl(const swf_block_desc* desc, const swf_block_stream_params* px,
                            const swf_block_stream_params* py, const float* x_in, const float* y_in, float* x_out,
                            float* y_out, int B, int H, int W, void* workspace, size_t workspace_bytes,
                            hipStream_t stream, const void* prepacked_x = nullptr, const void* prepacked_y = nullptr,
                            const void* next_x = nullptr, const void* next_y = nullptr, size_t next_bytes = 0,
                            const swf_block_stream_params* const* next_p = nullptr, bool* ln1_ready = nullptr, int* route = nullptr) {
    if (desc->precision == SWF_PREC_FAST && py && window_block_supported(*desc, B, H, W)) {
        if (ln1_ready) *ln1_ready = false;
        const bool prepacked = prepacked_x && prepacked_y;
        const size_t pb = window_block_packed_bytes(*desc);
        const size_t map_bytes = (size_t)B * H * W * desc->attn.channels * 4;
        const bool via_tmp = window_block_out_of_place(*desc) && desc->cross && (x_in == x_out || y_in == y_out || x_in == y_out || y_in == x_out);
        Carver ws(workspace, workspace_bytes);
        const WindowBufs bufs = carve_window_block(ws, *desc, (int64_t)B * H * W, prepacked, via_tmp);
        if (!ws.ok()) return fail(SWF_ERR_WORKSPACE, "fused block workspace too small (need %zu B)", ws.bytes());
        char* w = bufs.packed;
        float *ox = via_tmp ? bufs.ox : x_out, *oy = via_tmp ? bufs.oy : y_out;
        trace_block(route, SWF_BLOCK_ROUTE_WINDOW);
        if (prepacked) {
            SWF_TRY(launch_window_block(*desc, prepacked_x, prepacked_y, x_in, y_in, ox, oy, B, H, W, stream, next_x, next_y, next_bytes, route));
            trace_block(route, SWF_BLOCK_PREPACKED);
        } else {
            SWF_TRY(pack_window_block(*desc, *px, *py, w, w + pb, stream));
            SWF_TRY(launch_window_block(*desc, w, w + pb, x_in, y_in, ox, oy, B, H, W, stream, nullptr, nullptr, 0, route));
        }
        if (via_tmp) {
            trace_block(route, SWF_BLOCK_VIA_TMP);
            if (hipMemcpyAsync(x_out, ox, map_bytes, hipMemcpyDeviceToDevice, stream) != hipSuccess ||
                hipMemcpyAsync(y_out, oy, map_bytes, hipMemcpyDeviceToDevice, stream) != hipSuccess)
                return fail(SWF_ERR_HIP, "fused block: copy of the temporary outputs failed");
        }
        return SWF_OK;
    }
    auto aligned16 = [](const swf_block_stream_params* p) {
        if (!p) return true;
        const void* v[] = {p->ln1.gamma, p->ln1.beta, p->ln2.gamma, p->ln2.beta, p->attn.q.weight, p->attn.k.weight, p->attn.v.weight,
                           p->attn.proj.weight, p->fc1.weight, p->fc2.weight, p->attn.q.bias, p->attn.k.bias, p->attn.v.bias,
                           p->attn.proj.bias, p->fc1.bias, p->fc2.bias};
        uintptr_t bits = 0;
        for (const void* q : v) bits |= reinterpret_cast<uintptr_t>(q);
        return bits % 16 == 0;
    };
    const uintptr_t tbits = reinterpret_cast<uintptr_t>(x_in) | reinterpret_cast<uintptr_t>(y_in) | reinterpret_cast<uintptr_t>(x_out) |
                            reinterpret_cast<uintptr_t>(y_out);
    static const bool no_deep = debug_env("SWF_NO_DEEP") != nullptr;
    if (deep_block_supported(*desc) && !no_deep && tbits % 16 == 0 && aligned16(px) && aligned16(py)) {
        Carver ws(workspace, workspace_bytes);
        return deep_block_impl(desc, px, py, x_in, y_in, x_out, y_out, B, H, W, ws, stream, prepacked_x, prepacked_y, next_p, ln1_ready, route);
    }
    if (ln1_ready) *ln1_ready = false;
    trace_block(route, SWF_BLOCK_ROUTE_GENERIC);
    {
        Carver ws(workspace, workspace_bytes);
        SWF_TRY(attn_halfblock_generic(desc, px, py, x_in, y_in, x_out, y_out, B, H, W, ws, stream));
    }
    Carver ws(workspace, workspace_bytes);
    return mlp_halfblock_generic(desc, px, py, x_out, y_out, x_out, y_out, B, H, W, ws, stream);
}

static int pad_amount(int len, int mult) { return (mult - len % mult) % mult; }

static int merge_shapes(int H, int W, int mh, int mw, int wh, int ww, int* Hm, int* Wm, int* Ho, int* Wo) {
    if (H <= 0 || W <= 0 || mh <= 0 || mw <= 0 || wh <= 0 || ww <= 0) return fail(SWF_ERR_BAD_SHAPE, "non-positive size");
    const int ph = pad_amount(H, mh), pw = pad_amount(W, mw);
    if (ph >= H || pw >= W) return fail(SWF_ERR_PAD, "reflect pad (%d,%d) >= map (%d,%d) before merging", ph, pw, H, W);
    *Hm = (H + ph) / mh;
    *Wm = (W + pw) / mw;
    const int qh = pad_amount(*Hm, wh), qw = pad_amount(*Wm, ww);
    if (qh >= *Hm || qw >= *Wm)
        return fail(SWF_ERR_PAD, "Padding size should be less than the corresponding input dimension: pad (%d,%d) on a %dx%d map",
                    qh, qw, *Hm, *Wm);
    *Ho = *Hm + qh;
    *Wo = *Wm + qw;
    return SWF_OK;
}

static size_t patch_image_bytes(int decoder, int Cin, int Cout, int mh, int mw) {
    const size_t rr = patch_rr_packed_bytes(decoder, Cin, Cout, mh, mw);
    return rr ? rr : deep_patch_packed_bytes(decoder, Cin, Cout, mh, mw);
}
static int pack_patch_image(int decoder, int Cin, int Cout, int mh, int mw, const swf_patch_params& p, void* dst, hipStream_t stream) {
    if (patch_rr_packed_bytes(decoder, Cin, Cout, mh, mw))
        return pack_patch_rr(decoder, Cin, Cout, mh, mw, p.conv.weight, p.conv.bias, p.ln.gamma, p.ln.beta, dst, stream);
    return pack_deep_patch(decoder, Cin, Cout, mh, mw, p.conv.weight, dst, stream);
}

struct PatchTrace { int route; bf16_raw *ln_hi[2], *ln_lo[2]; };
static void trace_route(PatchTrace* t, int route) { if (t) t->route = route; }

struct DeepPatchBufs { bf16_raw *ln_hi[2], *ln_lo[2]; float* zr[2]; };
static DeepPatchBufs carve_deep_patch(Carver& ws, int nstream, bool with_ln, int64_t N_ln, int C_ln, int64_t row_floats) {
    DeepPatchBufs b{};
    if (with_ln) deep_ln1_planes(ws, N_ln, C_ln, nstream, b.ln_hi, b.ln_lo);
    for (int s = 0; s < nstream && row_floats; ++s) b.zr[s] = ws.floats(row_floats);
    return b;
}
static const DeepPatchExtra* deep_patch_ln(DeepPatchExtra& ex, const DeepPatchBufs& b, const swf_block_stream_params* const* blk, int nstream) {
    if (!blk) return nullptr;
    for (int s = 0; s < nstream; ++s) {
        ex.ln_gamma[s] = blk[s]->ln1.gamma; ex.ln_beta[s] = blk[s]->ln1.beta; ex.ln_hi[s] = b.ln_hi[s]; ex.ln_lo[s] = b.ln_lo[s];
    }
    return &ex;
}

struct PatchBufs { float *a[2], *z[2], *zn[2], *sk; int64_t sk_floats; };
static PatchBufs carve_merge_generic(Carver& ws, int nstream, int64_t N, int K, int Cout, int fast) {
    PatchBufs b{};
    for (int s = 0; s < nstream; ++s) { b.a[s] = ws.floats(N * K); b.z[s] = ws.floats(N * Cout); }
    b.sk_floats = fast ? splitk_need(K, nstream * N * Cout) : 0;
    b.sk = fast ? ws.floats(b.sk_floats) : nullptr;
    return b;
}
static PatchBufs carve_unmerge_generic(Carver& ws, int nstream, int64_t N, int Cin, int Kz, bool need_crop, int fast) {
    PatchBufs b{};
    for (int s = 0; s < nstream; ++s) {
        if (need_crop) b.a[s] = ws.floats(N * Cin);
        b.z[s] = ws.floats(N * Kz);
        b.zn[s] = ws.floats(N * Kz);
    }
    b.sk_floats = fast ? splitk_need(Cin, nstream * N * Kz) : 0;
    b.sk = fast ? ws.floats(b.sk_floats) : nullptr;
    return b;
}

static int patch_merge_impl(const swf_patch_params* const* p, int nstream, const float* const* in, float* const* out,
                            int B, int H, int W, int Cin, int Cout, int mh, int mw, int wh, int ww, void* workspace,
                            size_t workspace_bytes, hipStream_t stream, int fast = 0, const void* const* prr = nullptr,
                            const swf_block_stream_params* const* first_blk = nullptr, bool* ln1_ready = nullptr,
                            PatchTrace* trace = nullptr) {
    if (ln1_ready) *ln1_ready = false;
    int Hm, Wm, Ho, Wo;
    SWF_TRY(merge_shapes(H, W, mh, mw, wh, ww, &Hm, &Wm, &Ho, &Wo));
    const int64_t N = (int64_t)B * Ho * Wo;
    const int K = mh * mw * Cin;
    static const bool no_fused = debug_env("SWF_NO_FUSED_PATCH") != nullptr;
    static const bool no_prr = debug_env("SWF_NO_PATCH_RR") != nullptr;
    const bool use_prr = fast && !no_fused && !no_prr && prr && nstream == 2 && patch_rr_supported(0, Cin, Cout, mh, mw) &&
                         (int64_t)B * H * W * Cin < (int64_t(1) << 31);
    const bool use_dp = fast && !no_fused && !use_prr && prr && deep_patch_supported(0, Cin, Cout, mh, mw) && (int64_t)B * H * W * Cin < (int64_t(1) << 31);
    if (use_prr || use_dp || (fast && !no_fused && patch_fused_supported(K, Cout))) {
        PatchFusedDesc d{};
        for (int s = 0; s < nstream; ++s) {
            d.in[s] = in[s]; d.out[s] = out[s]; d.skip[s] = nullptr;
            d.w[s] = p[s]->conv.weight; d.bias[s] = p[s]->conv.bias; d.gamma[s] = p[s]->ln.gamma; d.beta[s] = p[s]->ln.beta;
        }
        d.decoder = 0; d.B = B; d.H = H; d.W = W; d.Cin = Cin; d.mh = mh; d.mw = mw; d.Hm = Hm; d.Wm = Wm; d.Ho = Ho; d.Wo = Wo;
        d.K = K; d.N = Cout; d.Cout = Cout; d.M = N;
        if (use_prr) { trace_route(trace, SWF_PATCH_ROUTE_RR); return launch_patch_rr(d, prr, nstream, stream); }
        if (use_dp) {
            const bool sliced = deep_patch_raw(0, Cin, Cout, mh, mw);
            const bool with_ln = first_blk && ln1_ready && first_blk[0] && (nstream == 1 || first_blk[1]) && (sliced || workspace);
            Carver wz(workspace, workspace_bytes);
            const DeepPatchBufs b = carve_deep_patch(wz, nstream, with_ln, N, Cout, sliced ? N * Cout : 0);
            if (!wz.ok()) return fail(SWF_ERR_WORKSPACE, "patch-merge workspace too small (need %zu B)", wz.bytes());
            DeepPatchExtra ex{};
            const DeepPatchExtra* ln = deep_patch_ln(ex, b, with_ln ? first_blk : nullptr, nstream);
            trace_route(trace, sliced ? SWF_PATCH_ROUTE_DEEP_SLICED : SWF_PATCH_ROUTE_DEEP_ROW);
            if (sliced) {
                SWF_TRY(launch_deep_patch(d, prr, nstream, stream, b.zr));
                SWF_TRY(launch_deep_patch_finish(d, b.zr, nstream, stream, ln));
            } else {
                SWF_TRY(launch_deep_patch(d, prr, nstream, stream, nullptr, ln));
            }
            if (with_ln) *ln1_ready = true;
            if (with_ln && trace) for (int s = 0; s < nstream; ++s) { trace->ln_hi[s] = b.ln_hi[s]; trace->ln_lo[s] = b.ln_lo[s]; }
            return SWF_OK;
        }
        trace_route(trace, SWF_PATCH_ROUTE_FUSED);
        return launch_patch_fused(d, nstream, stream);
    }
    trace_route(trace, SWF_PATCH_ROUTE_GENERIC);
    Carver ws(workspace, workspace_bytes);
    const PatchBufs bufs = carve_merge_generic(ws, nstream, N, K, Cout, fast);
    if (!ws.ok()) return fail(SWF_ERR_WORKSPACE, "patch-merge workspace too small (need %zu B)", ws.bytes());
    float* const *a = bufs.a, *const *z = bufs.z;
    PtrPair pp{};
    GemmBatch gb{};
    gb.scratch = bufs.sk; gb.scratch_floats = bufs.sk_floats;
    LnBatch lb{};
    for (int s = 0; s < nstream; ++s) {
        pp.in[s] = in[s]; pp.out[s] = a[s];
        gb.p[s] = GemmProb{a[s], p[s]->conv.weight, p[s]->conv.bias, nullptr, z[s]};
        lb.p[s] = LnProb{z[s], out[s], p[s]->ln.gamma, p[s]->ln.beta};
    }
    SWF_TRY(launch_merge_gather(pp, nstream, B, H, W, Cin, mh, mw, Hm, Wm, Ho, Wo, stream));
    SWF_TRY(launch_gemm(fast, gb, nstream, (int)N, Cout, K, K, Cout, 0, stream));
    return launch_layernorm(lb, nstream, N, Cout, 1, stream);
}

static int unmerge_shapes(int Hp, int Wp, int Hm, int Wm, int mh, int mw, int Hout, int Wout) {
    if (Hm <= 0 || Wm <= 0 || Hm > Hp || Wm > Wp) return fail(SWF_ERR_BAD_SHAPE, "crop %dx%d of %dx%d", Hm, Wm, Hp, Wp);
    if (Hout <= 0 || Wout <= 0 || Hout > Hm * mh || Wout > Wm * mw)
        return fail(SWF_ERR_BAD_SHAPE, "output %dx%d larger than the unmerged map %dx%d", Hout, Wout, Hm * mh, Wm * mw);
    return SWF_OK;
}

static int patch_unmerge_impl(const swf_patch_params* const* p, int nstream, const float* const* in,
                              const float* const* skip, float* const* out, int B, int Hp, int Wp, int Hm, int Wm, int Cin,
                              int Cout, int mh, int mw, int Hout, int Wout, void* workspace, size_t workspace_bytes,
                              hipStream_t stream, int fast = 0, const void* const* prr = nullptr, const char* warm = nullptr,
                              size_t warm_pb = 0, bool* warmed = nullptr, const swf_block_stream_params* const* next_blk = nullptr,
                              bool* ln1_ready = nullptr, PatchTrace* trace = nullptr) {
    if (ln1_ready) *ln1_ready = false;
    if (warmed) *warmed = false;
    SWF_TRY(unmerge_shapes(Hp, Wp, Hm, Wm, mh, mw, Hout, Wout));
    const int64_t N = (int64_t)B * Hm * Wm;
    const int Kz = mh * mw * Cout;
    const bool need_crop = (Hm != Hp) || (Wm != Wp);
    static const bool no_fused = debug_env("SWF_NO_FUSED_PATCH") != nullptr;
    static const bool no_prr = debug_env("SWF_NO_PATCH_RR") != nullptr;
    const bool use_prr = fast && !no_fused && !no_prr && prr && nstream == 2 && patch_rr_supported(1, Cin, Cout, mh, mw) &&
                         (int64_t)B * Hp * Wp * Cin < (int64_t(1) << 31);
    const bool use_dp = fast && !no_fused && !use_prr && prr && deep_patch_supported(1, Cin, Cout, mh, mw) && (int64_t)B * Hp * Wp * Cin < (int64_t(1) << 31);
    if (use_prr || use_dp || (fast && !no_fused && patch_fused_supported(Cin, Kz))) {
        PatchFusedDesc d{};
        for (int s = 0; s < nstream; ++s) {
            d.in[s] = in[s]; d.out[s] = out[s]; d.skip[s] = skip ? skip[s] : nullptr;
            d.w[s] = p[s]->conv.weight; d.bias[s] = p[s]->conv.bias; d.gamma[s] = p[s]->ln.gamma; d.beta[s] = p[s]->ln.beta;
        }
        d.decoder = 1; d.B = B; d.H = Hp; d.W = Wp; d.Cin = Cin; d.mh = mh; d.mw = mw; d.Hm = Hm; d.Wm = Wm; d.Ho = Hout; d.Wo = Wout;
        d.K = Cin; d.N = Kz; d.Cout = Cout; d.M = N;
        if (use_prr) { trace_route(trace, SWF_PATCH_ROUTE_RR); return launch_patch_rr(d, prr, nstream, stream); }
        if (use_dp && deep_patch_raw(1, Cin, Cout, mh, mw)) {
            const bool with_ln = next_blk && ln1_ready && next_blk[0] && (nstream == 1 || next_blk[1]);
            Carver wz(workspace, workspace_bytes);
            const DeepPatchBufs b = carve_deep_patch(wz, nstream, with_ln, (int64_t)B * Hout * Wout, Cout, N * Kz);
            if (!wz.ok()) return fail(SWF_ERR_WORKSPACE, "patch-unmerge workspace too small (need %zu B)", wz.bytes());
            DeepPatchExtra ex{};
            trace_route(trace, SWF_PATCH_ROUTE_DEEP_SLICED);
            SWF_TRY(launch_deep_patch(d, prr, nstream, stream, b.zr));
            SWF_TRY(launch_deep_patch_finish(d, b.zr, nstream, stream, deep_patch_ln(ex, b, with_ln ? next_blk : nullptr, nstream)));
            if (with_ln) *ln1_ready = true;
            if (with_ln && trace) for (int s = 0; s < nstream; ++s) { trace->ln_hi[s] = b.ln_hi[s]; trace->ln_lo[s] = b.ln_lo[s]; }
// ... 1638 lines not shown
```

Before: 9542 pairs/s.

## Finish projection, residual and LN2 inside the window attention kernel

Under the throughput schedule with the projection folded in, the qkv-attention kernel now runs one workgroup per window covering both head groups. It keeps the projection results in registers, adds the residual and projection bias, and writes x1 plus LN2-normalised bf16 hi/lo planes directly. The fused MLP kernel then loads those precomputed planes instead of re-reading the two fp32 partials and recomputing LayerNorm, which removes the partial-buffer round trip and the duplicated normalisation. In exchange the attention grid has half as many workgroups, each doing more work with an extra barrier between groups, and the path only covers C=192, 64-token tiles.

```diff
diff --git a/swin_unet_image_fusion_amd/csrc/kernels_mlp.h b/swin_unet_image_fusion_amd/csrc/kernels_mlp.h
--- a/swin_unet_image_fusion_amd/csrc/kernels_mlp.h
+++ b/swin_unet_image_fusion_amd/csrc/kernels_mlp.h
@@ -15,6 +15,7 @@
     int schedule;
     const float* ln_gamma[2]; const float* ln_beta[2]; bf16_raw* ln_hi[2]; bf16_raw* ln_lo[2];
     const float* part0[2]; const float* part1[2]; const float* pbias[2]; float* x1[2];
+    const bf16_raw* xn_hi[2]; const bf16_raw* xn_lo[2];
 };
 
 bool mlp_fused_supported(int C, int HID);
diff --git a/swin_unet_image_fusion_amd/csrc/kernels_mlp.hip b/swin_unet_image_fusion_amd/csrc/kernels_mlp.hip
--- a/swin_unet_image_fusion_amd/csrc/kernels_mlp.hip
+++ b/swin_unet_image_fusion_amd/csrc/kernels_mlp.hip
@@ -30,6 +30,7 @@
     int M, HID, splits, nchunks;
     const float* ln_gamma[2]; const float* ln_beta[2]; bf16* ln_hi[2]; bf16* ln_lo[2];
     const float* part0[2]; const float* part1[2]; const float* pbias[2]; float* x1[2];
+    const bf16* xn_hi[2]; const bf16* xn_lo[2];
 };
 
 __device__ __forceinline__ void mma3(f32x16& acc, const bf16x8 wh, const bf16x8 wl, const bf16x8 bh, const bf16x8 bl) {
@@ -100,7 +101,30 @@
 
     SWF_PROBE(0);
     const int hb0 = split * a.nchunks * CW;
-    {
+    bool planes = false;
+    if constexpr (C == 192 && NW == 4 && TOK == 64) planes = a.xn_hi[s] != nullptr;
+    if (planes) {
+        const int row = tid / TPR, sub = tid % TPR;
+        const int m = min(tile * TOK + row, a.M - 1);
+        constexpr int NCH = C / (8 * TPR);
+        const bf16* ph = a.xn_hi[s] + (int64_t)m * C;
+        const bf16* pl = a.xn_lo[s] + (int64_t)m * C;
+        u32x4 vh[NCH], vl[NCH];
+#pragma unroll
+        for (int i = 0; i < NCH; ++i) {
+            vh[i] = *reinterpret_cast<const u32x4*>(ph + 8 * (sub + TPR * i));
+            vl[i] = *reinterpret_cast<const u32x4*>(pl + 8 * (sub + TPR * i));
+        }
+        __builtin_amdgcn_sched_barrier(0);
+#pragma unroll
+        for (int f = 0; f < D; ++f) frag_load(f, hb0);
+        __builtin_amdgcn_sched_barrier(0);
+#pragma unroll
+        for (int i = 0; i < NCH; ++i) {
+            *reinterpret_cast<u32x4*>(a_hi + row * LDA + 8 * (sub + TPR * i)) = vh[i];
+            *reinterpret_cast<u32x4*>(a_lo + row * LDA + 8 * (sub + TPR * i)) = vl[i];
+        }
+    } else {
         const bool rowt = tid < LNT;
         const int row = rowt ? tid / TPR : 0, sub = tid % TPR;
         const int m = min(tile * TOK + row, a.M - 1);
@@ -319,7 +343,7 @@
     float4 exr[ENV], eb2[ENV], eg[ENV], ebt[ENV];
     const bool ln_out = !part && a.ln_hi[s] != nullptr;
     if (live) {
-        const float* xres = (a.part0[s] ? a.x1[s] : a.x[s]) + (int64_t)em * C;
+        const float* xres = (a.x1[s] ? a.x1[s] : a.x[s]) + (int64_t)em * C;
 #pragma unroll
         for (int i = 0; i < ENV; ++i) {
             const int c = ECS * i + 4 * esub;
@@ -504,7 +528,7 @@
     if (a.splits > 1) trace_block(route, SWF_BLOCK_MLP_SPLIT);
     MlpArgs ra = a;
     for (int s = 0; s < nstream; ++s)
-        if (a.part0[s]) ra.x[s] = a.x1[s];
+        if (a.x1[s]) ra.x[s] = a.x1[s];
     if (a.splits > 1 && a.ln_hi[0]) {
         constexpr int chunks = C / 4, L = chunks > 32 ? 64 : 32, NCH = (chunks + L - 1) / L;
         dim3 rgrid((unsigned)cdiv64((int64_t)a.M * L, 256), nstream);
@@ -562,6 +586,15 @@
             a.part0[s] = d.part0[s]; a.part1[s] = d.part1[s]; a.pbias[s] = d.pbias[s]; a.x1[s] = d.x1[s];
         }
     }
+    if (d.xn_hi[0]) {
+        if (d.part0[0] || d.C != 192 || d.schedule != SWF_SCHED_THROUGHPUT)
+            return fail(SWF_ERR_UNSUPPORTED, "mlp_fused: LN2 planes are taken by the 64-token C = 192 kernel of the throughput schedule, without partials");
+        for (int s = 0; s < nstream; ++s) {
+            if (!d.xn_hi[s] || !d.xn_lo[s] || !d.x1[s]) return fail(SWF_ERR_NULL, "mlp_fused: LN2 planes and x1 must be given for every stream");
+            if (d.x1[s] == d.out[s]) return fail(SWF_ERR_UNSUPPORTED, "mlp_fused: x1 must not alias out");
+            a.xn_hi[s] = reinterpret_cast<const bf16*>(d.xn_hi[s]); a.xn_lo[s] = reinterpret_cast<const bf16*>(d.xn_lo[s]); a.x1[s] = d.x1[s];
+        }
+    }
     a.M = d.M; a.HID = d.HID;
     a.splits = mlp_fused_splits(d.C, d.HID);
     const bool wide = mlp_wide(d.C, d.HID), tok32 = mlp_tok32(d.C, d.HID) && d.schedule != SWF_SCHED_THROUGHPUT;
diff --git a/swin_unet_image_fusion_amd/csrc/kernels_qkvattn.h b/swin_unet_image_fusion_amd/csrc/kernels_qkvattn.h
--- a/swin_unet_image_fusion_amd/csrc/kernels_qkvattn.h
+++ b/swin_unet_image_fusion_amd/csrc/kernels_qkvattn.h
@@ -12,6 +12,8 @@
     const bf16_raw* xn_hi[2]; const bf16_raw* xn_lo[2];
     bf16_raw* o_hi[2]; bf16_raw* o_lo[2];
     float* part[2][2];
+    bool rows;
+    const float* x[2]; const float* pbias[2]; const float* ln2_gamma[2]; const float* ln2_beta[2]; float* x1[2];
     int B, H, W, shift, cross;
 };
 int launch_qkvattn(const swf_block_desc& d, const QkvAttnArgs& a, int nstream, hipStream_t stream);
diff --git a/swin_unet_image_fusion_amd/csrc/kernels_qkvattn.hip b/swin_unet_image_fusion_amd/csrc/kernels_qkvattn.hip
--- a/swin_unet_image_fusion_amd/csrc/kernels_qkvattn.hip
+++ b/swin_unet_image_fusion_amd/csrc/kernels_qkvattn.hip
@@ -30,6 +30,7 @@
     const bf16* xn_hi[2]; const bf16* xn_lo[2];
     bf16* o_hi[2]; bf16* o_lo[2];
     float* part[2][2];
+    const float* x[2]; const float* pbias[2]; const float* ln2_gamma[2]; const float* ln2_beta[2]; float* x1[2];
     int B, H, W, shift, cross, nstream;
 };
 
@@ -40,11 +41,12 @@
 #define QA_STAMP(i) do { } while (0)
 #endif
 
-template <int C, int WS>
+template <int C, int WS, bool ROWS = false>
 __global__ __launch_bounds__(512, 2) void qkv_attn_kernel(QaDev a) {
     using G = QA<C>;
     static_assert(WS == 7 || WS == 8, "window side");
     constexpr int KS = G::KS, XS = G::XS;
+    constexpr int NG = ROWS ? G::HEADS / G::HG : 1;
     extern __shared__ __attribute__((aligned(16))) char smem[];
     u32x4* kimg = reinterpret_cast<u32x4*>(smem + G::l_k);
     u32x4* vimg = reinterpret_cast<u32x4*>(smem + G::l_v);
@@ -52,7 +54,8 @@
     const int tid = threadIdx.x, lane = tid & 63, wave = tid >> 6;
     const int hl = wave >> 1, tt = wave & 1, r = lane & 31, hf = lane >> 5;
     const int H = a.H, W = a.W, nwx = W / WS, nwy = H / WS, npi = nwx * nwy;
-    const int win = blockIdx.x, st = blockIdx.y, hg = blockIdx.z, head = hg * G::HG + hl;
+    const int win = blockIdx.x, st = blockIdx.y;
+    int hg = ROWS ? 0 : (int)blockIdx.z, head = hg * G::HG + hl;
     const int b = win / npi, wrem = win - b * npi, wy = wrem / nwx, wx = wrem - wy * nwx;
     const int sh = a.shift ? WS / 2 : 0;
     const bool cross = a.cross && a.nstream == 2;
@@ -68,16 +71,19 @@
     QA_STAMP(0);
     const __amdgpu_buffer_rsrc_t wrs = __builtin_amdgcn_make_buffer_rsrc(const_cast<char*>(uniform_ptr(a.packed[st])), 0, (int)G::p_total, 0x00020000);
     const unsigned loff = (unsigned)lane * 16u;
-    const int fbase = head * 3 * KS * 2;
+    int fbase = head * 3 * KS * 2;
     auto WFRAG = [&](int m, int s, int hl2) {
         return __builtin_bit_cast(u32x4, __builtin_amdgcn_raw_buffer_load_b128(wrs, loff, ((fbase + (m * KS + s) * 2 + hl2)) * 1024, 0));
     };
     constexpr int PD = 4;
     u32x4 w[PD][6];
-#pragma unroll
-    for (int p = 0; p < PD && p < KS; ++p)
-#pragma unroll
-        for (int m = 0; m < 3; ++m) { w[p][2 * m] = WFRAG(m, p, 0); w[p][2 * m + 1] = WFRAG(m, p, 1); }
+    auto ring_fill = [&] {
+#pragma unroll
+        for (int p = 0; p < PD && p < KS; ++p)
+#pragma unroll
+            for (int m = 0; m < 3; ++m) { w[p][2 * m] = WFRAG(m, p, 0); w[p][2 * m + 1] = WFRAG(m, p, 1); }
+    };
+    ring_fill();
 
     {
         constexpr int CPR = C / 8, NCH = 2 * 64 * CPR, PER = NCH / 512;
@@ -105,185 +111,299 @@
     const char* xq = smem + G::l_xq + (32 * tt + r) * XS + hf * 16;
     const char* xk = smem + (cross ? G::l_xkv : G::l_xq) + (32 * tt + r) * XS + hf * 16;
     const f32x16 zero16 = {0.f, 0.f, 0.f, 0.f, 0.f, 0.f, 0.f, 0.f, 0.f, 0.f, 0.f, 0.f, 0.f, 0.f, 0.f, 0.f};
-    f32x16 aq = zero16, ak = zero16, av = zero16;
-    {
-#pragma unroll
-        for (int s = 0; s < KS; ++s) {
-            SWF_WF_FENCE();
-            const u32x4 xh = *reinterpret_cast<const u32x4*>(xq + s * 32), xl = *reinterpret_cast<const u32x4*>(xq + G::l_plane + s * 32);
-            u32x4 kh = xh, kl = xl;
-            if (cross) {
-                kh = *reinterpret_cast<const u32x4*>(xk + s * 32);
-                kl = *reinterpret_cast<const u32x4*>(xk + G::l_plane + s * 32);
-            }
-            u32x4 (&ws_)[6] = w[s % PD];
-            aq = mma3(ws_[0], ws_[1], xh, xl, aq);
-            ak = mma3(ws_[2], ws_[3], kh, kl, ak);
-            av = mma3(kh, kl, ws_[4], ws_[5], av);
-            SWF_WF_FENCE();
-            if (s + PD < KS) {
-#pragma unroll
-                for (int m = 0; m < 3; ++m) { ws_[2 * m] = WFRAG(m, s + PD, 0); ws_[2 * m + 1] = WFRAG(m, s + PD, 1); }
-            }
-        }
-    }
-    QA_STAMP(2);
-    u32x4 qf[2];
-    {
-        const float* bvec = reinterpret_cast<const float*>(a.packed[st] + G::p_bvec) + head * 3 * 32;
-        float t[16];
-#pragma unroll
-        for (int g = 0; g < 4; ++g) {
-            const float4 bq = *reinterpret_cast<const float4*>(bvec + 8 * g + 4 * hf);
-            t[4 * g] = aq[4 * g] + bq.x; t[4 * g + 1] = aq[4 * g + 1] + bq.y; t[4 * g + 2] = aq[4 * g + 2] + bq.z; t[4 * g + 3] = aq[4 * g + 3] + bq.w;
-        }
-        qf[0] = pack8_f16(t);
-        qf[1] = pack8_f16(t + 8);
-#pragma unroll
-        for (int g = 0; g < 4; ++g) {
-            const float4 bk = *reinterpret_cast<const float4*>(bvec + 32 + 8 * g + 4 * hf);
-            t[4 * g] = ak[4 * g] + bk.x; t[4 * g + 1] = ak[4 * g + 1] + bk.y; t[4 * g + 2] = ak[4 * g + 2] + bk.z; t[4 * g + 3] = ak[4 * g + 3] + bk.w;
-        }
-        u32x4* kdst = kimg + ((hl * 2 + tt) * 2) * 64 + lane;
-        kdst[0] = pack8_f16(t);
-        kdst[64] = pack8_f16(t + 8);
-        const float bv = bvec[64 + r];
-#pragma unroll
-        for (int i = 0; i < 16; ++i) t[i] = av[i] + bv;
-        u32x4* vdst = vimg + (hl * 4 + 2 * tt) * 64 + lane;
-        vdst[0] = pack8_f16(t);
-        vdst[64] = pack8_f16(t + 8);
-    }
-    __syncthreads();
-    QA_STAMP(3);
-
-    const int qt = tt;
-    f32x16 bias[2];
-    {
-        const float* bm = reinterpret_cast<const float*>(a.packed[st] + G::p_bias) + qt * 2 * 16 * 64 + lane;
-#pragma unroll
-        for (int kt = 0; kt < 2; ++kt)
-#pragma unroll
-            for (int i = 0; i < 16; ++i) bias[kt][i] = bm[(kt * 16 + i) * 64];
-    }
-    const bool rowv = a.shift && wy == nwy - 1, colv = a.shift && wx == nwx - 1;
-    const bool col_masked = (hf != 0) != (((r >> 2) & 1) != 0);
-    const bool m0 = (rowv && qt == 1) || (colv && col_masked), m1 = (rowv && qt == 0) || (colv && col_masked);
-    const u32x4* ksrc = kimg + (hl * 4) * 64 + lane;
-    const u32x4* vsrc = vimg + (hl * 4) * 64 + lane;
-    const u32x4 k00 = ksrc[0], k01 = ksrc[64], k10 = ksrc[128], k11 = ksrc[192];
-    f32x16 s0 = mfma_f16(k00, qf[0], bias[0]);
-    s0 = mfma_f16(k01, qf[1], s0);
-    f32x16 s1 = mfma_f16(k10, qf[0], bias[1]);
-    s1 = mfma_f16(k11, qf[1], s1);
-    if (rowv || colv) {
-#pragma unroll
-        for (int i = 0; i < 16; ++i) {
-            s0[i] = m0 ? -INFINITY : s0[i];
-            s1[i] = m1 ? -INFINITY : s1[i];
-        }
-    }
-    float mx = max3f(s0[0], s0[1], s1[0]);
-    mx = max3f(mx, s1[1], s0[2]);
-#pragma unroll
-    for (int i = 3; i < 16; i += 2) mx = max3f(mx, s0[i], s0[i + 1 < 16 ? i + 1 : i]);
-#pragma unroll
-    for (int i = 2; i < 16; i += 2) mx = max3f(mx, s1[i], s1[i + 1]);
-    {
-        float lo, hi;
-        halves(mx, lo, hi);
-        mx = __builtin_fmaxf(lo, hi);
-    }
-    {
-        const f16 nm = (f16)(-mx);
-        u32x4 q1 = qf[1];
-        q1[2] |= hf == 0 ? (unsigned)__builtin_bit_cast(unsigned short, nm) : 0u;
-        s0 = mfma_f16(k00, qf[0], bias[0]);
-        s0 = mfma_f16(k01, q1, s0);
-        s1 = mfma_f16(k10, qf[0], bias[1]);
-        s1 = mfma_f16(k11, q1, s1);
-    }
-    if (rowv || colv) {
-#pragma unroll
-        for (int i = 0; i < 16; ++i) {
-            s0[i] = m0 ? -INFINITY : s0[i];
-            s1[i] = m1 ? -INFINITY : s1[i];
-        }
-    }
-    f32x16 t;
-#pragma unroll
-    for (int ps = 0; ps < 4; ++ps) {
-        float p[8];
-#pragma unroll
-        for (int j = 0; j < 8; ++j) p[j] = __builtin_amdgcn_exp2f((ps >> 1) ? s1[8 * (ps & 1) + j] : s0[8 * (ps & 1) + j]);
-        t = mfma_f16(vsrc[ps * 64], pack8_f16(p), ps == 0 ? zero16 : t);
-    }
-    QA_STAMP(4);
-    float den, unused;
-    halves(t[12], den, unused);
-    const float inv = __builtin_amdgcn_rcpf(den);
     auto padding = [](int t) { return WS != 8 && ((t >> 3) >= WS || (t & 7) >= WS); };
-    if (a.part[0][st] == nullptr) {
-        if (padding(32 * qt + r)) return;
-        const int64_t orow = (int64_t)tok_index(32 * qt + r) * (G::HEADS * G::D) + head * G::D + 4 * hf;
-        bf16* oh = a.o_hi[st] + orow;
-        bf16* ol = a.o_lo[st] + orow;
-#pragma unroll
-        for (int g = 0; g < 3; ++g) {
-            bf16x4 h4, l4;
-#pragma unroll
-            for (int j = 0; j < 4; ++j) {
-                const float v = t[4 * g + j] * inv;
-                h4[j] = (bf16)v;
-                l4[j] = (bf16)(v - (float)h4[j]);
-            }
-            *reinterpret_cast<bf16x4*>(oh + 8 * g) = h4;
-            *reinterpret_cast<bf16x4*>(ol + 8 * g) = l4;
-        }
-    } else {
+    constexpr int NJ = (G::NT + G::HG - 1) / G::HG;
+    constexpr int ORS = C + 4;
+    static_assert(size_t(64) * ORS * 4 <= G::l_tile, "the finished rows must fit the staging tile");
+    f32x16 keep[NJ];
+#pragma unroll
+    for (int grp = 0; grp < NG; ++grp) {
+        if (grp) { hg = grp; head = hg * G::HG + hl; }
+        f32x16 aq = zero16, ak = zero16, av = zero16;
+        {
+#pragma unroll
+            for (int s = 0; s < KS; ++s) {
+                SWF_WF_FENCE();
+                const u32x4 xh = *reinterpret_cast<const u32x4*>(xq + s * 32), xl = *reinterpret_cast<const u32x4*>(xq + G::l_plane + s * 32);
+                u32x4 kh = xh, kl = xl;
+                if (cross) {
+                    kh = *reinterpret_cast<const u32x4*>(xk + s * 32);
+                    kl = *reinterpret_cast<const u32x4*>(xk + G::l_plane + s * 32);
+                }
+                u32x4 (&ws_)[6] = w[s % PD];
+                aq = mma3(ws_[0], ws_[1], xh, xl, aq);
+                ak = mma3(ws_[2], ws_[3], kh, kl, ak);
+                av = mma3(kh, kl, ws_[4], ws_[5], av);
+                SWF_WF_FENCE();
+                if (s + PD < KS) {
+#pragma unroll
+                    for (int m = 0; m < 3; ++m) { ws_[2 * m] = WFRAG(m, s + PD, 0); ws_[2 * m + 1] = WFRAG(m, s + PD, 1); }
+                }
+            }
+        }
+        QA_STAMP(2);
+        u32x4 qf[2];
+        {
+            const float* bvec = reinterpret_cast<const float*>(a.packed[st] + G::p_bvec) + head * 3 * 32;
+            float t[16];
+#pragma unroll
+            for (int g = 0; g < 4; ++g) {
+                const float4 bq = *reinterpret_cast<const float4*>(bvec + 8 * g + 4 * hf);
+                t[4 * g] = aq[4 * g] + bq.x; t[4 * g + 1] = aq[4 * g + 1] + bq.y; t[4 * g + 2] = aq[4 * g + 2] + bq.z; t[4 * g + 3] = aq[4 * g + 3] + bq.w;
+            }
+            qf[0] = pack8_f16(t);
+            qf[1] = pack8_f16(t + 8);
+#pragma unroll
+            for (int g = 0; g < 4; ++g) {
+                const float4 bk = *reinterpret_cast<const float4*>(bvec + 32 + 8 * g + 4 * hf);
+                t[4 * g] = ak[4 * g] + bk.x; t[4 * g + 1] = ak[4 * g + 1] + bk.y; t[4 * g + 2] = ak[4 * g + 2] + bk.z; t[4 * g + 3] = ak[4 * g + 3] + bk.w;
+            }
+            if (ROWS && grp > 0) __syncthreads();
+            u32x4* kdst = kimg + ((hl * 2 + tt) * 2) * 64 + lane;
+            kdst[0] = pack8_f16(t);
+            kdst[64] = pack8_f16(t + 8);
+            const float bv = bvec[64 + r];
+#pragma unroll
+            for (int i = 0; i < 16; ++i) t[i] = av[i] + bv;
+            u32x4* vdst = vimg + (hl * 4 + 2 * tt) * 64 + lane;
+            vdst[0] = pack8_f16(t);
+            vdst[64] = pack8_f16(t + 8);
+        }
+        __syncthreads();
+        QA_STAMP(3);
+
+        const int qt = tt;
+        f32x16 bias[2];
+        {
+            const float* bm = reinterpret_cast<const float*>(a.packed[st] + G::p_bias) + qt * 2 * 16 * 64 + lane;
+#pragma unroll
+            for (int kt = 0; kt < 2; ++kt)
+#pragma unroll
+                for (int i = 0; i < 16; ++i) bias[kt][i] = bm[(kt * 16 + i) * 64];
+        }
+        const bool rowv = a.shift && wy == nwy - 1, colv = a.shift && wx == nwx - 1;
+        const bool col_masked = (hf != 0) != (((r >> 2) & 1) != 0);
+        const bool m0 = (rowv && qt == 1) || (colv && col_masked), m1 = (rowv && qt == 0) || (colv && col_masked);
+        const u32x4* ksrc = kimg + (hl * 4) * 64 + lane;
+        const u32x4* vsrc = vimg + (hl * 4) * 64 + lane;
+        const u32x4 k00 = ksrc[0], k01 = ksrc[64], k10 = ksrc[128], k11 = ksrc[192];
+        f32x16 s0 = mfma_f16(k00, qf[0], bias[0]);
+        s0 = mfma_f16(k01, qf[1], s0);
+        f32x16 s1 = mfma_f16(k10, qf[0], bias[1]);
+        s1 = mfma_f16(k11, qf[1], s1);
+        if (rowv || colv) {
+#pragma unroll
+            for (int i = 0; i < 16; ++i) {
+                s0[i] = m0 ? -INFINITY : s0[i];
+                s1[i] = m1 ? -INFINITY : s1[i];
+            }
+        }
+        float mx = max3f(s0[0], s0[1], s1[0]);
+        mx = max3f(mx, s1[1], s0[2]);
+#pragma unroll
+        for (int i = 3; i < 16; i += 2) mx = max3f(mx, s0[i], s0[i + 1 < 16 ? i + 1 : i]);
+#pragma unroll
+        for (int i = 2; i < 16; i += 2) mx = max3f(mx, s1[i], s1[i + 1]);
+        {
+            float lo, hi;
+            halves(mx, lo, hi);
+            mx = __builtin_fmaxf(lo, hi);
+        }
+        {
+            const f16 nm = (f16)(-mx);
+            u32x4 q1 = qf[1];
+            q1[2] |= hf == 0 ? (unsigned)__builtin_bit_cast(unsigned short, nm) : 0u;
+            s0 = mfma_f16(k00, qf[0], bias[0]);
+            s0 = mfma_f16(k01, q1, s0);
+            s1 = mfma_f16(k10, qf[0], bias[1]);
+            s1 = mfma_f16(k11, q1, s1);
+        }
         constexpr int NT = G::NT;
+        const bool last = ROWS && grp == NG - 1;
         const int pbase = (int)(G::p_proj / 1024) + hg * NT * G::HG * 4;
         auto PFRAG = [&](int tile, int f) {
             return __builtin_bit_cast(u32x4, __builtin_amdgcn_raw_buffer_load_b128(wrs, loff, (pbase + tile * G::HG * 4 + f) * 1024, 0));
         };
         u32x4 wp[G::HG * 4];
-#pragma unroll
-        for (int f = 0; f < G::HG * 4; ++f) wp[f] = PFRAG(hl, f);
-        float ov[16];
-#pragma unroll
-        for (int i = 0; i < 16; ++i) ov[i] = t[i] * inv;
-        u32x4* ofr = reinterpret_cast<u32x4*>(smem + G::l_xq);
-        {
-            u32x4 h0, l0, h1, l1;
-            split8(ov, h0, l0);
-            split8(ov + 8, h1, l1);
-            u32x4* dst = ofr + ((hl * 2 + tt) * 4) * 64 + lane;
-            dst[0] = h0; dst[64] = l0; dst[128] = h1; dst[192] = l1;
+        int tokrow[16];
+#pragma unroll
+        for (int i = 0; i < 16; ++i) tokrow[i] = tok_index(32 * tt + rho(i, hf)) * C;
+        if (ROWS && !last) {
+            SWF_WF_FENCE();
+            fbase = ((grp + 1) * G::HG + hl) * 3 * KS * 2;
+            ring_fill();
+            SWF_WF_FENCE();
+        }
+        if (rowv || colv) {
+#pragma unroll
+            for (int i = 0; i < 16; ++i) {
+                s0[i] = m0 ? -INFINITY : s0[i];
+                s1[i] = m1 ? -INFINITY : s1[i];
+            }
+        }
+        f32x16 t;
+#pragma unroll
+        for (int ps = 0; ps < 4; ++ps) {
+            float p[8];
+#pragma unroll
+            for (int j = 0; j < 8; ++j) p[j] = __builtin_amdgcn_exp2f((ps >> 1) ? s1[8 * (ps & 1) + j] : s0[8 * (ps & 1) + j]);
+            t = mfma_f16(vsrc[ps * 64], pack8_f16(p), ps == 0 ? zero16 : t);
+        }
+        QA_STAMP(4);
+        float den, unused;
+        halves(t[12], den, unused);
+        const float inv = __builtin_amdgcn_rcpf(den);
+        if (!ROWS && a.part[0][st] == nullptr) {
+            if (padding(32 * qt + r)) return;
+            const int64_t orow = (int64_t)tok_index(32 * qt + r) * (G::HEADS * G::D) + head * G::D + 4 * hf;
+            bf16* oh = a.o_hi[st] + orow;
+            bf16* ol = a.o_lo[st] + orow;
+#pragma unroll
+            for (int g = 0; g < 3; ++g) {
+                bf16x4 h4, l4;
+#pragma unroll
+                for (int j = 0; j < 4; ++j) {
+                    const float v = t[4 * g + j] * inv;
+                    h4[j] = (bf16)v;
+                    l4[j] = (bf16)(v - (float)h4[j]);
+                }
+                *reinterpret_cast<bf16x4*>(oh + 8 * g) = h4;
+                *reinterpret_cast<bf16x4*>(ol + 8 * g) = l4;
+            }
+        } else {
+            static_assert(!ROWS || NG == 2, "the rows-finishing shape keeps exactly one earlier partial");
+#pragma unroll
+            for (int f = 0; f < G::HG * 4; ++f) wp[f] = PFRAG(hl, f);
+            float xv[NJ][16], pb[NJ];
+            if (last) {
+#pragma unroll
+            for (int j = 0; j < NJ; ++j) {
+                const int tile = hl + G::HG * j;
+                pb[j] = 0.f;
+#pragma unroll
+                for (int i = 0; i < 16; ++i) xv[j][i] = 0.f;
+                if (tile < NT) {
+                    pb[j] = a.pbias[st][32 * tile + r];
+#pragma unroll
+                    for (int i = 0; i < 16; ++i) xv[j][i] = a.x[st][tokrow[i] + 32 * tile + r];
+                }
+            }
+            }
+            float ov[16];
+#pragma unroll
+            for (int i = 0; i < 16; ++i) ov[i] = t[i] * inv;
+            if (ROWS) __syncthreads();
+            u32x4* ofr = reinterpret_cast<u32x4*>(smem + (ROWS ? G::l_k : G::l_xq));
+            {
+                u32x4 h0, l0, h1, l1;
+                split8(ov, h0, l0);
+                split8(ov + 8, h1, l1);
+                u32x4* dst = ofr + ((hl * 2 + tt) * 4) * 64 + lane;
+                dst[0] = h0; dst[64] = l0; dst[128] = h1; dst[192] = l1;
+            }
+            __syncthreads();
+            auto proj_tile = [&](int tile) {
+                f32x16 acc = zero16;
+#pragma unroll
+                for (int h2 = 0; h2 < G::HG; ++h2)
+#pragma unroll
+                    for (int ks = 0; ks < 2; ++ks) {
+                        const u32x4* src = ofr + ((h2 * 2 + tt) * 4 + 2 * ks) * 64 + lane;
+                        acc = mma3(src[0], src[64], wp[(h2 * 2 + ks) * 2], wp[(h2 * 2 + ks) * 2 + 1], acc);
+                    }
+                if (tile + G::HG < NT) {
+#pragma unroll
+                    for (int f = 0; f < G::HG * 4; ++f) wp[f] = PFRAG(tile + G::HG, f);
+                }
+                return acc;
+            };
+            if constexpr (!ROWS) {
+                float* pout = a.part[hg][st];
+                for (int tile = hl; tile < NT; tile += G::HG) {
+                    const f32x16 acc = proj_tile(tile);
+#pragma unroll
+                    for (int i = 0; i < 16; ++i)
+                        if (!padding(32 * tt + rho(i, hf))) pout[tokrow[i] + 32 * tile + r] = acc[i];
+                }
+            } else {
+                float* rows = reinterpret_cast<float*>(smem + G::l_xq);
+#pragma unroll
+                for (int j = 0; j < NJ; ++j) {
+                    const int tile = hl + G::HG * j;
+                    if (tile < NT) {
+                        const f32x16 acc = proj_tile(tile);
+                        if (!last) {
+                            keep[j] = acc;
+                        } else {
+#pragma unroll
+                            for (int i = 0; i < 16; ++i)
+                                rows[(32 * tt + rho(i, hf)) * ORS + 32 * tile + r] = ((xv[j][i] + pb[j]) + keep[j][i]) + acc[i];
+                        }
+                    }
+                }
+            }
+        }
+        QA_STAMP(5);
+    }
+    if constexpr (ROWS) {
+        constexpr int NV = C / 16;
+        const bool rowt = tid >= 256;
+        const int row = (tid & 255) >> 2, sub = tid & 3;
+        float4 gm[NV], bt[NV];
+        if (rowt) {
+#pragma unroll
+            for (int i = 0; i < NV; ++i) {
+                gm[i] = *reinterpret_cast<const float4*>(a.ln2_gamma[st] + 16 * i + 4 * sub);
+                bt[i] = *reinterpret_cast<const float4*>(a.ln2_beta[st] + 16 * i + 4 * sub);
+            }
         }
         __syncthreads();
-        int tokrow[16];
-#pragma unroll
-        for (int i = 0; i < 16; ++i) tokrow[i] = tok_index(32 * tt + rho(i, hf)) * C;
-        float* pout = a.part[hg][st];
-        for (int tile = hl; tile < NT; tile += G::HG) {
-            f32x16 acc = zero16;
-#pragma unroll
-            for (int h2 = 0; h2 < G::HG; ++h2)
-#pragma unroll
-                for (int ks = 0; ks < 2; ++ks) {
-                    const u32x4* src = ofr + ((h2 * 2 + tt) * 4 + 2 * ks) * 64 + lane;
-                    acc = mma3(src[0], src[64], wp[(h2 * 2 + ks) * 2], wp[(h2 * 2 + ks) * 2 + 1], acc);
-                }
-            if (tile + G::HG < NT) {
-#pragma unroll
-                for (int f = 0; f < G::HG * 4; ++f) wp[f] = PFRAG(tile + G::HG, f);
-            }
-#pragma unroll
-            for (int i = 0; i < 16; ++i)
-                if (!padding(32 * tt + rho(i, hf))) pout[tokrow[i] + 32 * tile + r] = acc[i];
-        }
-    }
-    QA_STAMP(5);
+        if (rowt) {
+            const float* rows = reinterpret_cast<const float*>(smem + G::l_xq) + row * ORS;
+            const bool wr = !padding(row);
+            const int64_t grow = (int64_t)tok_index(row) * C;
+            float4 v[NV];
+#pragma unroll
+            for (int i = 0; i < NV; ++i) {
+                v[i] = *reinterpret_cast<const float4*>(rows + 16 * i + 4 * sub);
+                if (wr) *reinterpret_cast<float4*>(a.x1[st] + grow + 16 * i + 4 * sub) = v[i];
+            }
+            float sum = 0.f;
+#pragma unroll
+            for (int i = 0; i < NV; ++i) sum += (v[i].x + v[i].y) + (v[i].z + v[i].w);
+            sum += __shfl_xor(sum, 1);
+            sum += __shfl_xor(sum, 2);
+            constexpr int LN2_FUSED_MEAN = 7;
+            constexpr float RC = 1.0f / C;
+            float mean = sum * RC;
+            asm volatile("" : "+v"(mean));
+            float var = 0.f;
+#pragma unroll
+            for (int i = 0; i < NV; ++i) {
+                const float e[4] = {v[i].x, v[i].y, v[i].z, v[i].w};
+                float d[4];
+#pragma unroll
+                for (int j = 0; j < 4; ++j) d[j] = i < LN2_FUSED_MEAN ? __builtin_fmaf(sum, -RC, e[j]) : e[j] - mean;
+                var += __builtin_fmaf(d[0], d[0], d[1] * d[1]) + __builtin_fmaf(d[2], d[2], d[3] * d[3]);
+            }
+            var += __shfl_xor(var, 1);
+            var += __shfl_xor(var, 2);
+            const float rstd = 1.0f / sqrtf(__builtin_fmaf(var, RC, 1e-5f));
+            if (wr) {
+#pragma unroll
+                for (int i = 0; i < NV; ++i) {
+                    const int c = 16 * i + 4 * sub;
+                    const float n[4] = {__builtin_fmaf((v[i].x - mean) * rstd, gm[i].x, bt[i].x), __builtin_fmaf((v[i].y - mean) * rstd, gm[i].y, bt[i].y),
+                                        __builtin_fmaf((v[i].z - mean) * rstd, gm[i].z, bt[i].z), __builtin_fmaf((v[i].w - mean) * rstd, gm[i].w, bt[i].w)};
+                    bf16x4 h, l;
+#pragma unroll
+                    for (int j = 0; j < 4; ++j) { h[j] = (bf16)n[j]; l[j] = (bf16)(n[j] - (float)h[j]); }
+                    *reinterpret_cast<bf16x4*>(a.o_hi[st] + grow + c) = h;
+                    *reinterpret_cast<bf16x4*>(a.o_lo[st] + grow + c) = l;
+                }
+            }
+        }
+    }
 }
 
 struct QaPackArgs { swf_attn_params p; char* dst; int ws; };
@@ -367,7 +487,20 @@
         return fail(SWF_ERR_NULL, "qkvattn: projection partial buffers must be given for both head groups and streams or not at all");
     dv.B = a.B; dv.H = a.H; dv.W = a.W; dv.shift = a.shift; dv.cross = a.cross; dv.nstream = nstream;
     const int nwin = a.B * (a.H / wsd) * (a.W / wsd);
-    if (wsd == 8) {
+    if (a.rows) {
+        for (int s = 0; s < nstream; ++s) {
+            if (!a.x[s] || !a.pbias[s] || !a.ln2_gamma[s] || !a.ln2_beta[s] || !a.x1[s] || !a.o_hi[s] || !a.o_lo[s])
+                return fail(SWF_ERR_NULL, "qkvattn: the rows-finishing shape needs x, the projection bias, LN2 and x1 of every stream");
+            dv.x[s] = a.x[s]; dv.pbias[s] = a.pbias[s]; dv.ln2_gamma[s] = a.ln2_gamma[s]; dv.ln2_beta[s] = a.ln2_beta[s]; dv.x1[s] = a.x1[s];
+        }
+        if (wsd == 8) {
+            SWF_TRY((raise_lds_limit<&qkv_attn_kernel<192, 8, true>>((int)G::l_total, "qkv_attn")));
+            hipLaunchKernelGGL((qkv_attn_kernel<192, 8, true>), dim3(nwin, nstream, 1), dim3(512), G::l_total, stream, dv);
+        } else {
+            SWF_TRY((raise_lds_limit<&qkv_attn_kernel<192, 7, true>>((int)G::l_total, "qkv_attn")));
+            hipLaunchKernelGGL((qkv_attn_kernel<192, 7, true>), dim3(nwin, nstream, 1), dim3(512), G::l_total, stream, dv);
+        }
+    } else if (wsd == 8) {
         SWF_TRY((raise_lds_limit<&qkv_attn_kernel<192, 8>>((int)G::l_total, "qkv_attn")));
         hipLaunchKernelGGL((qkv_attn_kernel<192, 8>), dim3(nwin, nstream, 2), dim3(512), G::l_total, stream, dv);
     } else {
diff --git a/swin_unet_image_fusion_amd/csrc/swf_api.hip b/swin_unet_image_fusion_amd/csrc/swf_api.hip
--- a/swin_unet_image_fusion_amd/csrc/swf_api.hip
+++ b/swin_unet_image_fusion_amd/csrc/swf_api.hip
@@ -291,6 +291,7 @@
     if (!ws.ok()) return fail(SWF_ERR_WORKSPACE, "deep block workspace too small (need %zu B)", ws.bytes());
     static const bool no_qkvattn = debug_env("SWF_NO_QKVATTN") != nullptr;
     static const bool no_projfuse = debug_env("SWF_NO_PROJFUSE") != nullptr;
+    static const bool no_rowfinish = debug_env("SWF_NO_ROWFINISH") != nullptr;
     const bool fused_attn_shape = !no_qkvattn && qkvattn_supported(*desc) && N <= INT32_MAX / 256;
     const bool proj_fused = fused_attn_shape && fused_mlp && !no_projfuse && HD == C && (int64_t)H * W <= 256;
     DeepWeights wv[2];
@@ -309,12 +310,17 @@
     }
     const bool fused_attn = fused_attn_shape && wv[0].qa && (nstream == 1 || wv[1].qa);
     const bool fold_proj = proj_fused && fused_attn && pp[0]->attn.proj.bias && (nstream == 1 || pp[1]->attn.proj.bias);
+    const bool row_finish = fold_proj && desc->schedule == SWF_SCHED_THROUGHPUT && !no_rowfinish;
     if (fused_attn) {
         QkvAttnArgs qa{};
         for (int s = 0; s < nstream; ++s) {
             qa.packed[s] = wv[s].qa; qa.xn_hi[s] = b.xn_hi[s]; qa.xn_lo[s] = b.xn_lo[s]; qa.o_hi[s] = b.o_hi[s]; qa.o_lo[s] = b.o_lo[s];
-            if (fold_proj) { qa.part[0][s] = b.part[0][s]; qa.part[1][s] = b.part[1][s]; }
+            if (row_finish) {
+                qa.x[s] = xin[s]; qa.pbias[s] = pp[s]->attn.proj.bias; qa.ln2_gamma[s] = pp[s]->ln2.gamma; qa.ln2_beta[s] = pp[s]->ln2.beta;
+                qa.x1[s] = b.x1[s];
+            } else if (fold_proj) { qa.part[0][s] = b.part[0][s]; qa.part[1][s] = b.part[1][s]; }
         }
+        qa.rows = row_finish;
         qa.B = B; qa.H = H; qa.W = W; qa.shift = desc->attn.shift; qa.cross = cross;
         SWF_TRY(launch_qkvattn(*desc, qa, nstream, stream));
         trace_block(route, SWF_BLOCK_DEEP_QKVATTN | (fold_proj ? SWF_BLOCK_DEEP_FOLD_PROJ : 0));
@@ -389,7 +395,8 @@
         MlpFusedDesc md{};
         for (int s = 0; s < nstream; ++s) {
             md.x[s] = fold_proj ? xin[s] : xout[s]; md.out[s] = xout[s]; md.gamma[s] = pp[s]->ln2.gamma; md.beta[s] = pp[s]->ln2.beta;
-            if (fold_proj) { md.part0[s] = b.part[0][s]; md.part1[s] = b.part[1][s]; md.pbias[s] = pp[s]->attn.proj.bias; md.x1[s] = b.x1[s]; }
+            if (row_finish) { md.xn_hi[s] = b.o_hi[s]; md.xn_lo[s] = b.o_lo[s]; md.x1[s] = b.x1[s]; }
+            else if (fold_proj) { md.part0[s] = b.part[0][s]; md.part1[s] = b.part[1][s]; md.pbias[s] = pp[s]->attn.proj.bias; md.x1[s] = b.x1[s]; }
             md.w1_hi[s] = wv[s].w1f_hi; md.w1_lo[s] = wv[s].w1f_lo; md.w2_hi[s] = wv[s].w2f_hi; md.w2_lo[s] = wv[s].w2f_lo;
             md.b1[s] = pp[s]->fc1.bias; md.b2[s] = pp[s]->fc2.bias;
         }
```

Result: slower. 9385 pairs/s (-1.6%).
